# lucidrains/transfusion-pytorch

Hardware: NVIDIA H100
Metric: train tokens/sec (text+latent) at d=512 L=8 seq=1024 (higher is better)
Workload: dtype bf16

## Files before the change

transfusion_pytorch_b200/csrc/gemm_sm90.cuh:

```cuda
#pragma once
#include "sm90_ptx.cuh"
#include "dropout.cuh"

namespace tfx {

constexpr int GEMM_BM = 128;
constexpr int GEMM_BN = 128;
constexpr int GEMM_BK = 64;
constexpr int GEMM_UK = 16;

enum : int { EPI_STORE = 0, EPI_QKVG = 1, EPI_RESID = 2, EPI_GEGLU = 3, EPI_GEGLU_DROP = 4 };

struct GemmParams {
  int M, N, K;
  int k_splits;
  float* out_f32; long long ld_f32;
  __nv_bfloat16* out_bf16; long long ld_bf16;
  const float* bias;
  const long long* row_off;
  float alpha;
  int accumulate_f32;
  int K1;
  int H;
  __nv_bfloat16 *q, *k, *v;
  float* gates;
  float* mix_pre;
  float* qk_inv;
  const float *q_gamma, *k_gamma;
  const int* rope_pos;
  const float2* rope_cs;
  int rope_len;
  const int* kv_rows;
  const float* x_res; float* x_out; __nv_bfloat16* x_out_bf16;
  __nv_bfloat16* y_bf16;
  const int* cond_row;
  const float* zgate;
  long long zgate_ld;
  const float* ls;
  __nv_bfloat16* vg;
  __nv_bfloat16* h;
  DropParams drop;
};

template <int EPI> struct GemmCfg {
  static constexpr int THREADS = 384;
  static constexpr int STAGES = 4;
  static constexpr int A_BYTES = GEMM_BM * GEMM_BK * 2;
  static constexpr int B_BYTES = GEMM_BN * GEMM_BK * 2;
  static constexpr int STAGE_BYTES = A_BYTES + B_BYTES;
  static constexpr int ACC_BYTES = GEMM_BM * GEMM_BN * 4;
  static constexpr int STG_WARP = EPI == 2 ? 4096 + 2048 : 4096;
  static constexpr int STAGING = (EPI >= 3 ? 8 : 4) * STG_WARP;
  static constexpr int SMEM_BYTES = STAGES * STAGE_BYTES + ACC_BYTES + STAGING + 1024  + 256 ;
  static_assert(SMEM_BYTES <= 227 * 1024, "shared memory of one block");
};

__device__ __forceinline__ uint32_t acc_off(int r, int col) { return r * 512 + ((((col >> 2) ^ (r & 7))) << 4) + (col & 3) * 4; }
__device__ __forceinline__ void acc_ld32(const uint8_t* acc, int r, int col, uint32_t (&v)[32]) {
#pragma unroll
  for (int q = 0; q < 8; ++q) {
    const uint4 t = *reinterpret_cast<const uint4*>(acc + r * 512 + ((((col >> 2) + q) ^ (r & 7)) << 4));
    v[4 * q] = t.x; v[4 * q + 1] = t.y; v[4 * q + 2] = t.z; v[4 * q + 3] = t.w;
  }
}

__device__ __forceinline__ void gelu_parts(float g, float& cdf, float& pdf) {
  const float ax = fabsf(g) * 0.70710678118654752f;
  const float t = __fdividef(1.f, fmaf(0.3275911f, ax, 1.f));
  const float E = __expf(-ax * ax);
  float poly = fmaf(1.061405429f, t, -1.453152027f);
  poly = fmaf(poly, t, 1.421413741f);
  poly = fmaf(poly, t, -0.284496736f);
  poly = fmaf(poly, t, 0.254829592f);
  const float h = 0.5f * poly * t * E;
  cdf = g >= 0.f ? 1.f - h : h;
  pdf = 0.3989422804014327f * E;
}
__device__ __forceinline__ float gelu_erf(float x) { float c, d; gelu_parts(x, c, d); return x * c; }
__device__ __forceinline__ float2 geglu_pair(float2 g, float2 v) {
  return make_float2(gelu_erf(g.x) * v.x, gelu_erf(g.y) * v.y);
}

__device__ __forceinline__ void cp_async16_zfill(void* smem, const void* gmem, bool valid) {
  const int sz = valid ? 16 : 0;
  asm volatile("cp.async.cg.shared.global [%0], [%1], 16, %2;" ::"r"(smem_u32(smem)), "l"(gmem), "r"(sz) : "memory");
}

__device__ __forceinline__ uint32_t pack_bf16(float a, float b) {
  __nv_bfloat162 t = __floats2bfloat162_rn(a, b);
  return *reinterpret_cast<uint32_t*>(&t);
}
__device__ __forceinline__ float2 unpack2_bf16_(uint32_t w) {
  __nv_bfloat162 t = *reinterpret_cast<__nv_bfloat162*>(&w);
  return __bfloat1622float2(t);
}

template <int CH>
__device__ __forceinline__ void stg_put(uint8_t* sw, int lane, const uint32_t* w) {
#pragma unroll
  for (int c = 0; c < CH; ++c)
    *reinterpret_cast<uint4*>(sw + lane * 128 + ((c ^ (lane & 7)) << 4)) = make_uint4(w[4 * c], w[4 * c + 1], w[4 * c + 2], w[4 * c + 3]);
}
template <int CH>
__device__ __forceinline__ void stg_get(const uint8_t* sw, int lane, uint32_t* w) {
#pragma unroll
  for (int c = 0; c < CH; ++c) {
    const uint4 t = *reinterpret_cast<const uint4*>(sw + lane * 128 + ((c ^ (lane & 7)) << 4));
    w[4 * c] = t.x; w[4 * c + 1] = t.y; w[4 * c + 2] = t.z; w[4 * c + 3] = t.w;
  }
}
template <int CH>
__device__ __forceinline__ void stg_store(const uint8_t* sw, int lane, uint8_t* g, long long pitch, int rows_valid) {
  constexpr int RPI = 32 / CH;
#pragma unroll
  for (int it = 0; it < 32 / RPI; ++it) {
    const int row = it * RPI + lane / CH, ch = lane % CH;
    if (row < rows_valid)
      *reinterpret_cast<uint4*>(g + row * pitch + ch * 16) = *reinterpret_cast<const uint4*>(sw + row * 128 + ((ch ^ (row & 7)) << 4));
  }
}
__device__ __forceinline__ void stg_fetch(int lane, const uint8_t* g, long long pitch, int rows_valid, uint4 (&t)[8]) {
#pragma unroll
  for (int it = 0; it < 8; ++it) {
    const int row = it * 4 + lane / 8, ch = lane % 8;
    t[it] = row < rows_valid ? *reinterpret_cast<const uint4*>(g + row * pitch + ch * 16) : make_uint4(0, 0, 0, 0);
  }
}
__device__ __forceinline__ void stg_fill(uint8_t* sw, int lane, const uint4 (&t)[8]) {
#pragma unroll
  for (int it = 0; it < 8; ++it) {
    const int row = it * 4 + lane / 8, ch = lane % 8;
    *reinterpret_cast<uint4*>(sw + row * 128 + ((ch ^ (row & 7)) << 4)) = t[it];
  }
}

__device__ __forceinline__ void stg_put_pack(uint8_t* sw, int lane, const float* y) {
#pragma unroll
  for (int c = 0; c < 4; ++c)
    *reinterpret_cast<uint4*>(sw + lane * 128 + ((c ^ (lane & 7)) << 4)) =
        make_uint4(pack_bf16(y[8 * c], y[8 * c + 1]), pack_bf16(y[8 * c + 2], y[8 * c + 3]), pack_bf16(y[8 * c + 4], y[8 * c + 5]), pack_bf16(y[8 * c + 6], y[8 * c + 7]));
}
__device__ __forceinline__ void stg64_put(uint8_t* sw, int lane, const uint32_t* w) {
#pragma unroll
  for (int c = 0; c < 4; ++c)
    *reinterpret_cast<uint4*>(sw + lane * 64 + ((c ^ ((lane >> 1) & 3)) << 4)) = make_uint4(w[4 * c], w[4 * c + 1], w[4 * c + 2], w[4 * c + 3]);
}
__device__ __forceinline__ void stg64_put_pack(uint8_t* sw, int lane, const float* y) {
#pragma unroll
  for (int c = 0; c < 4; ++c)
    *reinterpret_cast<uint4*>(sw + lane * 64 + ((c ^ ((lane >> 1) & 3)) << 4)) =
        make_uint4(pack_bf16(y[8 * c], y[8 * c + 1]), pack_bf16(y[8 * c + 2], y[8 * c + 3]), pack_bf16(y[8 * c + 4], y[8 * c + 5]), pack_bf16(y[8 * c + 6], y[8 * c + 7]));
}
__device__ __forceinline__ void stg64_store(const uint8_t* sw, int lane, uint8_t* g, long long pitch, int rows_valid) {
#pragma unroll
  for (int it = 0; it < 4; ++it) {
    const int row = it * 8 + (lane >> 2), ch = lane & 3;
    if (row < rows_valid)
      *reinterpret_cast<uint4*>(g + row * pitch + ch * 16) = *reinterpret_cast<const uint4*>(sw + row * 64 + ((ch ^ ((row >> 1) & 3)) << 4));
  }
}

__device__ __forceinline__ void stg64_store_rows(const uint8_t* sw, int lane, uint8_t* g, long long pitch, int rows_valid, const int* __restrict__ rows) {
#pragma unroll
  for (int it = 0; it < 4; ++it) {
    const int row = it * 8 + (lane >> 2), ch = lane & 3;
    if (row < rows_valid)
      *reinterpret_cast<uint4*>(g + (long long)rows[row] * pitch + ch * 16) = *reinterpret_cast<const uint4*>(sw + row * 64 + ((ch ^ ((row >> 1) & 3)) << 4));
  }
}
template <int CH>
__device__ __forceinline__ void stg_store_rows(const uint8_t* sw, int lane, uint8_t* g, long long pitch, int rows_valid, const int* __restrict__ rows) {
  constexpr int RPI = 32 / CH;
#pragma unroll
  for (int it = 0; it < 32 / RPI; ++it) {
    const int row = it * RPI + lane / CH, ch = lane % CH;
    if (row < rows_valid)
      *reinterpret_cast<uint4*>(g + (long long)rows[row] * pitch + ch * 16) = *reinterpret_cast<const uint4*>(sw + row * 128 + ((ch ^ (row & 7)) << 4));
  }
}

template <bool A_MN, bool B_MN, int EPI, int CL>
__global__ void __launch_bounds__(384, 1)
gemm_sm90_kernel(const __grid_constant__ CUtensorMap tmA, const __grid_constant__ CUtensorMap tmA2, const __grid_constant__ CUtensorMap tmB, const GemmParams p) {
  using Cfg = GemmCfg<EPI>;
  constexpr bool GEGLU = EPI == EPI_GEGLU || EPI == EPI_GEGLU_DROP;
  constexpr int BN = GEMM_BN;
  constexpr int STAGES = Cfg::STAGES;
  static_assert(Cfg::STAGE_BYTES % 1024 == 0 && 2 * STAGES <= 32, "stage alignment / barrier area");
  extern __shared__ __align__(1024) uint8_t smem_raw[];
  uint8_t* smem = smem_raw;
  if (threadIdx.x == 0 && (smem_u32(smem) & 1023u) != 0) __trap();
  uint8_t* acc = smem + STAGES * Cfg::STAGE_BYTES;
  uint8_t* staging = acc + Cfg::ACC_BYTES;
  uint64_t* bars = reinterpret_cast<uint64_t*>(staging + Cfg::STAGING);
  uint64_t* full_bar = bars;
  uint64_t* empty_bar = bars + STAGES;

  const int warp = threadIdx.x >> 5, lane = threadIdx.x & 31;
  const int m_tiles = (p.M + GEMM_BM - 1) / GEMM_BM;
  const int n_tiles = (p.N + BN - 1) / BN;
  const int kb_total = (p.K + GEMM_BK - 1) / GEMM_BK;
  const int kb_per_split = (kb_total + p.k_splits - 1) / p.k_splits;
  const int m_units = (m_tiles + CL - 1) / CL;
  const int unit_items = m_units * n_tiles;
  const int num_items = unit_items * p.k_splits;
  const int cta_rank = CL > 1 ? (int)cluster_ctarank() : 0;
  const int first_item = blockIdx.x / CL, item_stride = gridDim.x / CL;

  if (threadIdx.x == 0) {
    tma_prefetch_desc(&tmA);
    tma_prefetch_desc(&tmB);
    for (int s = 0; s < STAGES; ++s) { mbar_init(&full_bar[s], 1); mbar_init(&empty_bar[s], 4 * CL); }
    mbar_fence_init();
  }
  __syncthreads();
  if constexpr (CL > 1) cluster_sync_all();

  if (warp < 4) {
    setmaxnreg_dec<40>();
    if (threadIdx.x == 0) {
      int stage = 0; uint32_t phase = 0;
      for (int item = first_item; item < num_items; item += item_stride) {
        const int split = item / unit_items;
        const int rem = item - split * unit_items;
        const int m_unit = rem / n_tiles, n_blk = rem - m_unit * n_tiles;
        const int m_blk = m_unit * CL + cta_rank;
        const int kb0 = split * kb_per_split;
        const int kb1 = min(kb0 + kb_per_split, kb_total);
        for (int kb = kb0; kb < kb1; ++kb) {
          mbar_wait(&empty_bar[stage], phase ^ 1);
          uint8_t* sA = smem + stage * Cfg::STAGE_BYTES;
          uint8_t* sB = sA + Cfg::A_BYTES;
          mbar_expect_tx(&full_bar[stage], Cfg::STAGE_BYTES);
          if (!A_MN) {
            if (kb * GEMM_BK < p.K1) tma_load_2d(&tmA, &full_bar[stage], sA, kb * GEMM_BK, m_blk * GEMM_BM);
            else tma_load_2d(&tmA2, &full_bar[stage], sA, kb * GEMM_BK - p.K1, m_blk * GEMM_BM);
          } else {
#pragma unroll
            for (int a = 0; a < GEMM_BM / 64; ++a)
              tma_load_2d(&tmA, &full_bar[stage], sA + a * (GEMM_BK * 128), m_blk * GEMM_BM + a * 64, kb * GEMM_BK);
          }
          if constexpr (CL > 1) {
            if (!B_MN) tma_load_2d_multicast(&tmB, &full_bar[stage], sB + cta_rank * (64 * 128), kb * GEMM_BK, n_blk * BN + cta_rank * 64, (uint16_t)3);
            else tma_load_2d_multicast(&tmB, &full_bar[stage], sB + cta_rank * (GEMM_BK * 128), n_blk * BN + cta_rank * 64, kb * GEMM_BK, (uint16_t)3);
          } else if (!B_MN) {
            tma_load_2d(&tmB, &full_bar[stage], sB, kb * GEMM_BK, n_blk * BN);
          } else {
#pragma unroll
            for (int a = 0; a < BN / 64; ++a)
              tma_load_2d(&tmB, &full_bar[stage], sB + a * (GEMM_BK * 128), n_blk * BN + a * 64, kb * GEMM_BK);
          }
          if (++stage == STAGES) { stage = 0; phase ^= 1; }
        }
      }
    }
  } else {
    setmaxnreg_inc<232>();
    constexpr int BAR_TILE = 1, BAR_MMA = 3, BAR_ACC = 5;
    const int cw = (warp >> 2) - 1;
    const int quad = warp & 3;
    uint8_t* sw = staging + ((GEGLU ? 4 * cw : 0) + quad) * Cfg::STG_WARP;
    const int erow = quad * 32 + lane;
    int stage = 0; uint32_t phase = 0;
    auto release = [&](int s) {
      __syncwarp();
      if (lane == 0) {
        if constexpr (CL > 1) { mbar_arrive_cluster(&empty_bar[s], 0); mbar_arrive_cluster(&empty_bar[s], 1); }
        else mbar_arrive(&empty_bar[s]);
      }
    };
    int nth = 0;
    for (int item = first_item; item < num_items; item += item_stride, ++nth) {
      const int split = item / unit_items;
      const int rem = item - split * unit_items;
      const int m_unit = rem / n_tiles, n_blk = rem - m_unit * n_tiles;
      const int m_blk = m_unit * CL + cta_rank;
      const int kb0 = split * kb_per_split;
      const int kb1 = min(kb0 + kb_per_split, kb_total);
      if ((nth & 1) != cw) {
        const int s = stage + (kb1 - kb0);
        stage = s % STAGES;
        phase ^= (uint32_t)(s / STAGES) & 1u;
        continue;
      }
      const bool has_next = item + item_stride < num_items;
      if (nth > 0) named_bar_sync(BAR_MMA + cw, 256);
      float d0[64], d1[64];
#pragma unroll
      for (int i = 0; i < 64; ++i) { d0[i] = 0.f; d1[i] = 0.f; }
      int prev_stage = -1;
      for (int kb = kb0; kb < kb1; ++kb) {
        mbar_wait(&full_bar[stage], phase);
        const uint32_t sA = smem_u32(smem + stage * Cfg::STAGE_BYTES);
        const uint32_t sB = sA + Cfg::A_BYTES;
        wgmma_reg_fence(d0);
        wgmma_reg_fence(d1);
        wgmma_fence();
#pragma unroll
        for (int k = 0; k < GEMM_BK / GEMM_UK; ++k) {
          const uint64_t db = B_MN ? wgmma_desc_sw128(sB + k * (GEMM_UK * 128), GEMM_BK * 128, 1024)
                                   : wgmma_desc_sw128(sB + k * (GEMM_UK * 2), 16, 1024);
          const uint64_t da0 = A_MN ? wgmma_desc_sw128(sA + k * (GEMM_UK * 128), GEMM_BK * 128, 1024)
                                    : wgmma_desc_sw128(sA + k * (GEMM_UK * 2), 16, 1024);
          const uint64_t da1 = A_MN ? wgmma_desc_sw128(sA + GEMM_BK * 128 + k * (GEMM_UK * 128), GEMM_BK * 128, 1024)
                                    : wgmma_desc_sw128(sA + 64 * 128 + k * (GEMM_UK * 2), 16, 1024);
          const uint32_t acc_flag = (kb > kb0 || k > 0) ? 1u : 0u;
          wgmma_m64n128_ss<A_MN ? 1 : 0, B_MN ? 1 : 0>(d0, da0, db, acc_flag);
          wgmma_m64n128_ss<A_MN ? 1 : 0, B_MN ? 1 : 0>(d1, da1, db, acc_flag);
        }
        wgmma_commit();
        wgmma_wait<1>();
        if (prev_stage >= 0) release(prev_stage);
        prev_stage = stage;
        if (++stage == STAGES) { stage = 0; phase ^= 1; }
      }
      if (has_next) named_bar_arrive(BAR_MMA + (cw ^ 1), 256);
      wgmma_wait<0>();
      wgmma_reg_fence(d0);
      wgmma_reg_fence(d1);
      if (prev_stage >= 0) release(prev_stage);

      if (nth > 0) named_bar_sync(BAR_ACC + cw, 256);
      {
        const int r0 = quad * 16 + (lane >> 2);
#pragma unroll
        for (int q = 0; q < 16; ++q) {
          const int c = 8 * q + 2 * (lane & 3);
          *reinterpret_cast<float2*>(acc + acc_off(r0, c)) = make_float2(d0[4 * q], d0[4 * q + 1]);
          *reinterpret_cast<float2*>(acc + acc_off(r0 + 8, c)) = make_float2(d0[4 * q + 2], d0[4 * q + 3]);
          *reinterpret_cast<float2*>(acc + acc_off(r0 + 64, c)) = make_float2(d1[4 * q], d1[4 * q + 1]);
          *reinterpret_cast<float2*>(acc + acc_off(r0 + 72, c)) = make_float2(d1[4 * q + 2], d1[4 * q + 3]);
        }
      }
      named_bar_sync(BAR_TILE + cw, 128);

      const int wrow0 = m_blk * GEMM_BM + quad * 32;
      const int row = wrow0 + lane;
      const bool row_ok = row < p.M;
      const int rows_valid = min(32, p.M - wrow0);
      const int col0 = n_blk * BN;
      int qk_pos = 0;
      if constexpr (EPI == EPI_QKVG) { qk_pos = row_ok ? p.rope_pos[row] : 0; }
      if constexpr (EPI == EPI_RESID) { qk_pos = (row_ok && p.cond_row) ? p.cond_row[row] : -1; }

      if constexpr (EPI == EPI_STORE) {
        const bool f32_staged = p.out_f32 && (p.row_off || (p.ld_f32 & 3) == 0) && ((reinterpret_cast<uintptr_t>(p.out_f32) & 15) == 0);
        const bool bf16_staged = p.out_bf16 && (p.ld_bf16 & 7) == 0 && ((reinterpret_cast<uintptr_t>(p.out_bf16) & 15) == 0);
#pragma unroll 1
        for (int c = 0; c < BN / 32; ++c) {
          const int cbase = col0 + c * 32;
          if (cbase >= p.N) break;
          uint32_t r[32];
          acc_ld32(acc, erow, c * 32, r);
          const bool full = cbase + 32 <= p.N;
          float v[32];
#pragma unroll
          for (int j = 0; j < 32; ++j) v[j] = __uint_as_float(r[j]);
          if (p.alpha != 1.f) {
#pragma unroll
            for (int j = 0; j < 32; ++j) v[j] *= p.alpha;
          }
          if (p.bias) {
            if (full) {
#pragma unroll
              for (int j = 0; j < 32; j += 4) { const float4 b = *reinterpret_cast<const float4*>(p.bias + cbase + j); v[j] += b.x; v[j + 1] += b.y; v[j + 2] += b.z; v[j + 3] += b.w; }
            } else {
              for (int j = 0; j < 32; ++j) if (cbase + j < p.N) v[j] += p.bias[cbase + j];
            }
          }
          if (p.out_f32) {
            if (full && f32_staged) {
#pragma unroll
              for (int j = 0; j < 32; ++j) r[j] = __float_as_uint(v[j]);
              stg_put<8>(sw, lane, r);
              __syncwarp();
#pragma unroll
              for (int it = 0; it < 8; ++it) {
                const int rr = it * 4 + (lane >> 3), ch = lane & 7;
                if (rr < rows_valid) {
                  const long long off = p.row_off ? p.row_off[wrow0 + rr] : (long long)(wrow0 + rr) * p.ld_f32;
                  if (off >= 0) {
                    float* dst = p.out_f32 + off + cbase + ch * 4;
                    const float4 t = *reinterpret_cast<const float4*>(sw + rr * 128 + ((ch ^ (rr & 7)) << 4));
                    if ((reinterpret_cast<uintptr_t>(dst) & 15) == 0) {
                      if (p.accumulate_f32) asm volatile("red.global.add.v4.f32 [%0], {%1, %2, %3, %4};" ::"l"(dst), "f"(t.x), "f"(t.y), "f"(t.z), "f"(t.w) : "memory");
                      else *reinterpret_cast<float4*>(dst) = t;
                    } else {
                      if (p.accumulate_f32) { atomicAdd(dst, t.x); atomicAdd(dst + 1, t.y); atomicAdd(dst + 2, t.z); atomicAdd(dst + 3, t.w); }
                      else { dst[0] = t.x; dst[1] = t.y; dst[2] = t.z; dst[3] = t.w; }
                    }
                  }
                }
              }
              __syncwarp();
            } else if (row_ok) {
              const long long off = p.row_off ? p.row_off[row] : (long long)row * p.ld_f32;
              if (off >= 0) {
                float* dst = p.out_f32 + off + cbase;
                for (int j = 0; j < 32; ++j)
                  if (cbase + j < p.N) { if (p.accumulate_f32) atomicAdd(dst + j, v[j]); else dst[j] = v[j]; }
              }
            }
          }
          if (p.out_bf16) {
            if (full && bf16_staged) {
              uint32_t w[16];
#pragma unroll
              for (int j = 0; j < 16; ++j) w[j] = pack_bf16(v[2 * j], v[2 * j + 1]);
              stg_put<4>(sw, lane, w);
              __syncwarp();
              stg_store<4>(sw, lane, reinterpret_cast<uint8_t*>(p.out_bf16 + (long long)wrow0 * p.ld_bf16 + cbase), p.ld_bf16 * 2, rows_valid);
              __syncwarp();
            } else if (row_ok) {
              __nv_bfloat16* dst = p.out_bf16 + (long long)row * p.ld_bf16 + cbase;
              for (int j = 0; j < 32; ++j) if (cbase + j < p.N) dst[j] = __float2bfloat16(v[j]);
            }
          }
        }
      } else if constexpr (EPI == EPI_QKVG) {
        const int tps = p.H >> 1;
        const int kind = n_blk / tps;
        const int tis = n_blk - kind * tps;
        const long long HI = (long long)p.H * 64;
        if (kind <= 1) {
          const float* gamma = kind == 0 ? p.q_gamma : p.k_gamma;
          __nv_bfloat16* dstm = kind == 0 ? p.q : p.k;
          const float2* cs = p.rope_cs + qk_pos;
#pragma unroll
          for (int hh = 0; hh < 2; ++hh) {
            uint32_t r0[32], r1[32];
            acc_ld32(acc, erow, hh * 64, r0);
            acc_ld32(acc, erow, hh * 64 + 32, r1);
            float ss = 0.f;
#pragma unroll
            for (int j = 0; j < 32; ++j) { float a = __uint_as_float(r0[j]), b = __uint_as_float(r1[j]); ss += a * a + b * b; }
            const float inv = 1.f / fmaxf(sqrtf(ss), 1e-12f);
            const int head = tis * 2 + hh;
            if (row_ok) p.qk_inv[(long long)row * 2 * p.H + kind * p.H + head] = inv;
            const float sc = inv * 8.f;
            uint32_t outw[32];
#pragma unroll
            for (int dh = 0; dh < 2; ++dh) {
              uint32_t* rr = dh == 0 ? r0 : r1;
#pragma unroll
              for (int i = 0; i < 16; ++i) {
                const int d0 = dh * 32 + 2 * i;
                const float2 gm = *reinterpret_cast<const float2*>(gamma + d0);
                const float y0 = __uint_as_float(rr[2 * i]) * sc * (gm.x + 1.f);
                const float y1 = __uint_as_float(rr[2 * i + 1]) * sc * (gm.y + 1.f);
                const float2 cc = cs[(long long)(dh * 16 + i) * p.rope_len];
                outw[dh * 16 + i] = pack_bf16(y0 * cc.x - y1 * cc.y, y1 * cc.x + y0 * cc.y);
              }
            }
            stg_put<8>(sw, lane, outw);
            __syncwarp();
            if (kind == 1 && p.kv_rows) stg_store_rows<8>(sw, lane, reinterpret_cast<uint8_t*>(dstm + head * 64), HI * 2, rows_valid, p.kv_rows + wrow0);
            else stg_store<8>(sw, lane, reinterpret_cast<uint8_t*>(dstm + (long long)wrow0 * HI + head * 64), HI * 2, rows_valid);
            __syncwarp();
          }
        } else if (kind == 2) {
#pragma unroll
          for (int c = 0; c < 2; ++c) {
            uint32_t r0[32], r1[32], w[32];
            acc_ld32(acc, erow, c * 64, r0);
            acc_ld32(acc, erow, c * 64 + 32, r1);
#pragma unroll
            for (int j = 0; j < 16; ++j) {
              w[j] = pack_bf16(__uint_as_float(r0[2 * j]), __uint_as_float(r0[2 * j + 1]));
              w[16 + j] = pack_bf16(__uint_as_float(r1[2 * j]), __uint_as_float(r1[2 * j + 1]));
            }
            stg_put<8>(sw, lane, w);
            __syncwarp();
            if (p.kv_rows) stg_store_rows<8>(sw, lane, reinterpret_cast<uint8_t*>(p.v + tis * 128 + c * 64), HI * 2, rows_valid, p.kv_rows + wrow0);
            else stg_store<8>(sw, lane, reinterpret_cast<uint8_t*>(p.v + (long long)wrow0 * HI + tis * 128 + c * 64), HI * 2, rows_valid);
            __syncwarp();
          }
        } else {
          uint32_t r[32];
          acc_ld32(acc, erow, 0, r);
          if (row_ok) {
            float* dst = p.gates + (long long)row * p.H;
#pragma unroll
            for (int j = 0; j < 32; ++j) if (j < p.H) dst[j] = __uint_as_float(r[j]);
            if (p.mix_pre) {
              float* dm = p.mix_pre + (long long)row * p.H;
#pragma unroll
              for (int j = 0; j < 32; ++j) if (j >= p.H && j < 2 * p.H) dm[j - p.H] = __uint_as_float(r[j]);
            }
          }
        }
      } else if constexpr (EPI == EPI_RESID) {
        const int crow = qk_pos;
        const float* zrow = (p.zgate && crow >= 0) ? p.zgate + (long long)crow * p.zgate_ld : nullptr;
        uint8_t* swb = sw + 4096;
        uint4 xres[8];
        auto fetch = [&](int sl) {
          stg_fetch(lane, reinterpret_cast<const uint8_t*>(p.x_res + (long long)wrow0 * p.N + col0 + sl * 32), (long long)p.N * 4,
                    col0 + sl * 32 < p.N ? rows_valid : 0, xres);
        };
        fetch(0);
#pragma unroll 1
        for (int sl = 0; sl < BN / 32; ++sl) {
          const int cbase = col0 + sl * 32;
          if (cbase >= p.N) break;
          __syncwarp();
          stg_fill(sw, lane, xres);
          if (sl + 1 < BN / 32) fetch(sl + 1);
          uint32_t r[32];
          acc_ld32(acc, erow, sl * 32, r);
          float y[32];
#pragma unroll
          for (int j = 0; j < 32; ++j) y[j] = __uint_as_float(r[j]);
          if (p.bias) {
#pragma unroll
            for (int j = 0; j < 32; j += 4) { const float4 b = *reinterpret_cast<const float4*>(p.bias + cbase + j); y[j] += b.x; y[j + 1] += b.y; y[j + 2] += b.z; y[j + 3] += b.w; }
          }
          if (p.y_bf16) {
            stg64_put_pack(swb, lane, y);
            __syncwarp();
            stg64_store(swb, lane, reinterpret_cast<uint8_t*>(p.y_bf16 + (long long)wrow0 * p.N + cbase), (long long)p.N * 2, rows_valid);
            __syncwarp();
          }
          {
            uint32_t xrv[32];
            __syncwarp();
            stg_get<8>(sw, lane, xrv);
            if (zrow) {
#pragma unroll
              for (int j = 0; j < 32; j += 4) {
                const float4 s4 = *reinterpret_cast<const float4*>(zrow + cbase + j);
                y[j] = __uint_as_float(xrv[j]) + y[j] * s4.x; y[j + 1] = __uint_as_float(xrv[j + 1]) + y[j + 1] * s4.y;
                y[j + 2] = __uint_as_float(xrv[j + 2]) + y[j + 2] * s4.z; y[j + 3] = __uint_as_float(xrv[j + 3]) + y[j + 3] * s4.w;
              }
            } else if (p.ls) {
#pragma unroll
              for (int j = 0; j < 32; j += 4) {
                const float4 s4 = *reinterpret_cast<const float4*>(p.ls + cbase + j);
                y[j] = __uint_as_float(xrv[j]) + y[j] * (s4.x + 1.f); y[j + 1] = __uint_as_float(xrv[j + 1]) + y[j + 1] * (s4.y + 1.f);
                y[j + 2] = __uint_as_float(xrv[j + 2]) + y[j + 2] * (s4.z + 1.f); y[j + 3] = __uint_as_float(xrv[j + 3]) + y[j + 3] * (s4.w + 1.f);
              }
            } else {
#pragma unroll
              for (int j = 0; j < 32; ++j) y[j] += __uint_as_float(xrv[j]);
            }
          }
          if (p.x_out)
#pragma unroll
          for (int hfc = 0; hfc < 2; ++hfc) {
            uint32_t w16[16];
#pragma unroll
            for (int j = 0; j < 16; ++j) w16[j] = __float_as_uint(y[hfc * 16 + j]);
            __syncwarp();
            stg64_put(swb, lane, w16);
            __syncwarp();
            stg64_store(swb, lane, reinterpret_cast<uint8_t*>(p.x_out + (long long)wrow0 * p.N + cbase + hfc * 16), (long long)p.N * 4, rows_valid);
          }
          if (p.x_out_bf16) {
            __syncwarp();
            stg64_put_pack(swb, lane, y);
            __syncwarp();
            stg64_store(swb, lane, reinterpret_cast<uint8_t*>(p.x_out_bf16 + (long long)wrow0 * p.N + cbase), (long long)p.N * 2, rows_valid);
          }
          __syncwarp();
        }
      } else if constexpr (GEGLU) {
        uint32_t keep[2] = {0u, 0u};
        if constexpr (EPI == EPI_GEGLU_DROP) {
          const uint32_t k0 = __ldg(p.drop.key), k1 = __ldg(p.drop.key + 1);
#pragma unroll
          for (int q = 0; q < 8; ++q) keep[q >> 2] |= drop_keep8(p.drop, k0, k1, DROP_SITE_FFN, 0, (uint32_t)row, (uint32_t)(n_blk * 8 + q)) << (8 * (q & 3));
        }
        uint32_t ra[4][32];
#pragma unroll
        for (int q = 0; q < 4; ++q) acc_ld32(acc, erow, q * 32, ra[q]);
        if (has_next) named_bar_arrive(BAR_ACC + (cw ^ 1), 256);
#pragma unroll
        for (int c = 0; c < 2; ++c) {
          const int cv = col0 + c * 32, cg = cv + 64;
          if (cv >= p.N) break;
          float v[32], g[32];
#pragma unroll
          for (int j = 0; j < 32; ++j) { v[j] = __uint_as_float(ra[c][j]) + p.bias[cv + j]; g[j] = __uint_as_float(ra[2 + c][j]) + p.bias[cg + j]; }
          __syncwarp();
          stg64_put_pack(sw, lane, v);
          __syncwarp();
          stg64_store(sw, lane, reinterpret_cast<uint8_t*>(p.vg + (long long)wrow0 * p.N + cv), (long long)p.N * 2, rows_valid);
          __syncwarp();
          stg64_put_pack(sw, lane, g);
          __syncwarp();
          stg64_store(sw, lane, reinterpret_cast<uint8_t*>(p.vg + (long long)wrow0 * p.N + cg), (long long)p.N * 2, rows_valid);
#pragma unroll
          for (int j = 0; j < 32; j += 2) {
            const float2 o = geglu_pair(make_float2(g[j], g[j + 1]), make_float2(v[j], v[j + 1]));
            g[j] = o.x; g[j + 1] = o.y;
          }
          if constexpr (EPI == EPI_GEGLU_DROP) {
#pragma unroll
            for (int j = 0; j < 32; ++j) g[j] = (keep[c] >> j) & 1u ? g[j] * p.drop.scale : 0.f;
          }
          __syncwarp();
          stg64_put_pack(sw, lane, g);
          __syncwarp();
          stg64_store(sw, lane, reinterpret_cast<uint8_t*>(p.h + (long long)wrow0 * (p.N / 2) + n_blk * 64 + c * 32), (long long)p.N, rows_valid);
          __syncwarp();
        }
      }
      if (!GEGLU && has_next) named_bar_arrive(BAR_ACC + (cw ^ 1), 256);
    }
  }
  if constexpr (CL > 1) {
    __syncthreads();
    cluster_sync_all();
  }
}

typedef CUresult (*PFN_encodeTiled)(CUtensorMap*, CUtensorMapDataType, cuuint32_t, void*, const cuuint64_t*, const cuuint64_t*,
                                    const cuuint32_t*, const cuuint32_t*, CUtensorMapInterleave, CUtensorMapSwizzle,
                                    CUtensorMapL2promotion, CUtensorMapFloatOOBfill);

inline PFN_encodeTiled get_encode_fn() {
  static PFN_encodeTiled fn = nullptr;
  if (!fn) {
    void* f = nullptr;
    cudaDriverEntryPointQueryResult qres;
    if (cudaGetDriverEntryPoint("cuTensorMapEncodeTiled", &f, cudaEnableDefault, &qres) != cudaSuccess || !f) return nullptr;
    fn = reinterpret_cast<PFN_encodeTiled>(f);
  }
  return fn;
}

inline int make_tmap_bf16(CUtensorMap* tm, const void* ptr, long long inner, long long outer, long long ld, int box_rows) {
  PFN_encodeTiled enc = get_encode_fn();
  if (!enc) return -1;
  cuuint64_t dims[2] = {(cuuint64_t)inner, (cuuint64_t)outer};
  cuuint64_t strides[1] = {(cuuint64_t)ld * 2};
  cuuint32_t box[2] = {64, (cuuint32_t)box_rows};
  cuuint32_t estr[2] = {1, 1};
  CUresult r = enc(tm, CU_TENSOR_MAP_DATA_TYPE_BFLOAT16, 2, const_cast<void*>(ptr), dims, strides, box, estr,
                   CU_TENSOR_MAP_INTERLEAVE_NONE, CU_TENSOR_MAP_SWIZZLE_128B, CU_TENSOR_MAP_L2_PROMOTION_L2_256B,
                   CU_TENSOR_MAP_FLOAT_OOB_FILL_NONE);
  return r == CUDA_SUCCESS ? 0 : -(int)r - 1000;
}

struct GemmOperand {
  const void* ptr;
  long long ld;
  bool mn_major;
  const void* ptr2 = nullptr;
  long long ld2 = 0;
};

inline int& gemm_cluster_mode_ref() {
  static int mode = -1;
  if (mode < 0) { const char* e = getenv("TFX_GEMM_CLUSTER"); mode = e ? atoi(e) : 1; }
  return mode;
}

template <bool A_MN, bool B_MN, int EPI>
int launch_gemm_t(const GemmOperand& A, const GemmOperand& B, const GemmParams& p_in, int num_sms, cudaStream_t stream) {
  using Cfg = GemmCfg<EPI>;
  GemmParams p = p_in;
  CUtensorMap tmA, tmA2, tmB;
  int rc;
  const bool two = (!A_MN) && A.ptr2 != nullptr;
  if (!two) p.K1 = p.K;
  if (!A_MN) rc = make_tmap_bf16(&tmA, A.ptr, two ? p.K1 : p.K, p.M, A.ld, GEMM_BM); else rc = make_tmap_bf16(&tmA, A.ptr, p.M, p.K, A.ld, GEMM_BK);
  if (rc) return rc;
  if (two) { rc = make_tmap_bf16(&tmA2, A.ptr2, p.K - p.K1, p.M, A.ld2, GEMM_BM); if (rc) return rc; } else tmA2 = tmA;
  {
    const int kbt = (p.K + GEMM_BK - 1) / GEMM_BK;
    if (p.k_splits < 1) p.k_splits = 1;
    if (p.k_splits > kbt) p.k_splits = kbt;
    const int per = (kbt + p.k_splits - 1) / p.k_splits;
    p.k_splits = (kbt + per - 1) / per;
  }
  const int m_tiles = (p.M + GEMM_BM - 1) / GEMM_BM, n_tiles = (p.N + GEMM_BN - 1) / GEMM_BN;
  const int items = m_tiles * n_tiles * p.k_splits;
  if (items <= 0) return 0;
  const int mode = gemm_cluster_mode_ref();
  const int kb_item = ((p.K + GEMM_BK - 1) / GEMM_BK + p.k_splits - 1) / p.k_splits;
  const bool paired = mode == 2 || (mode == 3 && m_tiles >= 2 && kb_item >= 16 && items >= 2 * num_sms);
  if (!B_MN) rc = make_tmap_bf16(&tmB, B.ptr, p.K, p.N, B.ld, paired ? GEMM_BN / 2 : GEMM_BN); else rc = make_tmap_bf16(&tmB, B.ptr, p.N, p.K, B.ld, GEMM_BK);
  if (rc) return rc;
  if (paired) {
    auto kern = gemm_sm90_kernel<A_MN, B_MN, EPI, 2>;
    static int max_clusters = 0;
    cudaLaunchConfig_t cfg;
    memset(&cfg, 0, sizeof(cfg));
    cudaLaunchAttribute at[1];
    at[0].id = cudaLaunchAttributeClusterDimension;
    at[0].val.clusterDim.x = 2; at[0].val.clusterDim.y = 1; at[0].val.clusterDim.z = 1;
    cfg.blockDim = dim3(Cfg::THREADS); cfg.dynamicSmemBytes = Cfg::SMEM_BYTES; cfg.stream = stream; cfg.attrs = at; cfg.numAttrs = 1;
    if (!max_clusters) {
      if (cudaFuncSetAttribute(kern, cudaFuncAttributeMaxDynamicSharedMemorySize, Cfg::SMEM_BYTES) != cudaSuccess) return -2;
      cfg.gridDim = dim3(2 * (num_sms / 2));
      int nc = 0;
      if (cudaOccupancyMaxActiveClusters(&nc, kern, &cfg) != cudaSuccess || nc < 1) { cudaGetLastError(); nc = num_sms / 2; }
      max_clusters = nc < num_sms / 2 ? nc : num_sms / 2;
    }
    const int pair_items = ((m_tiles + 1) / 2) * n_tiles * p.k_splits;
    const int clusters = pair_items < max_clusters ? pair_items : max_clusters;
    cfg.gridDim = dim3(2 * clusters);
    return cudaLaunchKernelEx(&cfg, kern, tmA, tmA2, tmB, p) == cudaSuccess ? 0 : -3;
  }
  auto kern = gemm_sm90_kernel<A_MN, B_MN, EPI, 1>;
  static bool attr_set = false;
  if (!attr_set) {
    if (cudaFuncSetAttribute(kern, cudaFuncAttributeMaxDynamicSharedMemorySize, Cfg::SMEM_BYTES) != cudaSuccess) return -2;
    attr_set = true;
  }
  const int grid = items < num_sms ? items : num_sms;
  kern<<<grid, Cfg::THREADS, Cfg::SMEM_BYTES, stream>>>(tmA, tmA2, tmB, p);
  return cudaGetLastError() == cudaSuccess ? 0 : -3;
}

}
```

transfusion_pytorch_b200/csrc/sm90_ptx.cuh:

```cuda
#pragma once
#include <cuda.h>
#include <cuda_runtime.h>
#include <cuda_bf16.h>
#include <stdint.h>
#include <stdio.h>

namespace tfx {

#ifndef TFX_SPIN_LIMIT
#define TFX_SPIN_LIMIT (1u << 24)
#endif

__device__ __forceinline__ uint32_t smem_u32(const void* p) {
  return static_cast<uint32_t>(__cvta_generic_to_shared(p));
}

__device__ __forceinline__ void mbar_init(uint64_t* bar, uint32_t count) {
  asm volatile("mbarrier.init.shared::cta.b64 [%0], %1;" ::"r"(smem_u32(bar)), "r"(count));
}
__device__ __forceinline__ void mbar_fence_init() {
  asm volatile("fence.mbarrier_init.release.cluster;" ::: "memory");
}
__device__ __forceinline__ void mbar_expect_tx(uint64_t* bar, uint32_t bytes) {
  asm volatile("mbarrier.arrive.expect_tx.shared::cta.b64 _, [%0], %1;" ::"r"(smem_u32(bar)), "r"(bytes) : "memory");
}
__device__ __forceinline__ void mbar_arrive(uint64_t* bar) {
  asm volatile("mbarrier.arrive.shared::cta.b64 _, [%0];" ::"r"(smem_u32(bar)) : "memory");
}
__device__ __forceinline__ bool mbar_try_wait(uint64_t* bar, uint32_t parity) {
  uint32_t ok;
  asm volatile(
      "{\n\t.reg .pred p;\n\t"
      "mbarrier.try_wait.parity.shared::cta.b64 p, [%1], %2;\n\t"
      "selp.u32 %0, 1, 0, p;\n\t}"
      : "=r"(ok) : "r"(smem_u32(bar)), "r"(parity) : "memory");
  return ok != 0;
}
__device__ __forceinline__ void mbar_wait(uint64_t* bar, uint32_t parity) {
  uint32_t spins = 0;
  while (!mbar_try_wait(bar, parity)) {
    if (++spins > TFX_SPIN_LIMIT) {
#if defined(TFX_DEBUG_SPIN) && TFX_DEBUG_SPIN
      printf("tfx: mbarrier timeout block %d thread %d bar %u parity %u\n", blockIdx.x, threadIdx.x, smem_u32(bar), parity);
#endif
      __trap();
    }
  }
}

__device__ __forceinline__ void tma_prefetch_desc(const CUtensorMap* m) {
  asm volatile("prefetch.tensormap [%0];" ::"l"(reinterpret_cast<uint64_t>(m)) : "memory");
}
__device__ __forceinline__ void tma_load_2d(const CUtensorMap* m, uint64_t* bar, void* smem, int c0, int c1) {
  asm volatile(
      "cp.async.bulk.tensor.2d.shared::cluster.global.mbarrier::complete_tx::bytes [%0], [%1, {%3, %4}], [%2];"
      ::"r"(smem_u32(smem)), "l"(reinterpret_cast<uint64_t>(m)), "r"(smem_u32(bar)), "r"(c0), "r"(c1)
      : "memory");
}
__device__ __forceinline__ void tma_load_1d(const CUtensorMap* m, uint64_t* bar, void* smem, int c0) {
  asm volatile(
      "cp.async.bulk.tensor.1d.shared::cluster.global.mbarrier::complete_tx::bytes [%0], [%1, {%3}], [%2];"
      ::"r"(smem_u32(smem)), "l"(reinterpret_cast<uint64_t>(m)), "r"(smem_u32(bar)), "r"(c0)
      : "memory");
}
__device__ __forceinline__ void tma_reduce_add_2d(const CUtensorMap* m, const void* smem, int c0, int c1) {
  asm volatile("cp.reduce.async.bulk.tensor.2d.global.shared::cta.add.tile.bulk_group [%0, {%2, %3}], [%1];"
               ::"l"(reinterpret_cast<uint64_t>(m)), "r"(smem_u32(smem)), "r"(c0), "r"(c1) : "memory");
}
__device__ __forceinline__ void bulk_commit() { asm volatile("cp.async.bulk.commit_group;" ::: "memory"); }
__device__ __forceinline__ void bulk_wait_read_all() { asm volatile("cp.async.bulk.wait_group.read 0;" ::: "memory"); }
__device__ __forceinline__ void bulk_wait_all() { asm volatile("cp.async.bulk.wait_group 0;" ::: "memory"); }
__device__ __forceinline__ void tma_load_2d_multicast(const CUtensorMap* m, uint64_t* bar, void* smem, int c0, int c1, uint16_t mask) {
  asm volatile(
      "cp.async.bulk.tensor.2d.shared::cluster.global.mbarrier::complete_tx::bytes.multicast::cluster [%0], [%1, {%3, %4}], [%2], %5;"
      ::"r"(smem_u32(smem)), "l"(reinterpret_cast<uint64_t>(m)), "r"(smem_u32(bar)), "r"(c0), "r"(c1), "h"(mask)
      : "memory");
}
__device__ __forceinline__ uint32_t cluster_ctarank() { uint32_t r; asm volatile("mov.u32 %0, %%cluster_ctarank;" : "=r"(r)); return r; }
__device__ __forceinline__ void cluster_sync_all() {
  asm volatile("barrier.cluster.arrive.release.aligned;\n\tbarrier.cluster.wait.acquire.aligned;" ::: "memory");
}
__device__ __forceinline__ void mbar_arrive_cluster(uint64_t* bar, uint32_t rank) {
  uint32_t remote;
  asm volatile("mapa.shared::cluster.u32 %0, %1, %2;" : "=r"(remote) : "r"(smem_u32(bar)), "r"(rank));
  asm volatile("mbarrier.arrive.release.cluster.shared::cluster.b64 _, [%0];" ::"r"(remote) : "memory");
}
__device__ __forceinline__ void fence_proxy_async_smem() {
  asm volatile("fence.proxy.async.shared::cta;" ::: "memory");
}
__device__ __forceinline__ void named_bar_sync(int id, int count) {
  asm volatile("bar.sync %0, %1;" ::"r"(id), "r"(count) : "memory");
}
__device__ __forceinline__ void named_bar_arrive(int id, int count) {
  asm volatile("bar.arrive %0, %1;" ::"r"(id), "r"(count) : "memory");
}

template <int N> __device__ __forceinline__ void setmaxnreg_dec() { asm volatile("setmaxnreg.dec.sync.aligned.u32 %0;" ::"n"(N)); }
template <int N> __device__ __forceinline__ void setmaxnreg_inc() { asm volatile("setmaxnreg.inc.sync.aligned.u32 %0;" ::"n"(N)); }

__device__ __forceinline__ void wgmma_fence() { asm volatile("wgmma.fence.sync.aligned;" ::: "memory"); }
__device__ __forceinline__ void wgmma_commit() { asm volatile("wgmma.commit_group.sync.aligned;" ::: "memory"); }
template <int N> __device__ __forceinline__ void wgmma_wait() { asm volatile("wgmma.wait_group.sync.aligned %0;" ::"n"(N) : "memory"); }
template <int N> __device__ __forceinline__ void wgmma_reg_fence(float (&d)[N]) {
#pragma unroll
  for (int i = 0; i < N; ++i) asm volatile("" : "+f"(d[i])::"memory");
}

template <int TA, int TB>
__device__ __forceinline__ void wgmma_m64n128_ss(float (&d)[64], uint64_t da, uint64_t db, uint32_t accumulate) {
  asm volatile(
      "{\n\t.reg .pred p;\n\t"
      "setp.ne.b32 p, %66, 0;\n\t"
      "wgmma.mma_async.sync.aligned.m64n128k16.f32.bf16.bf16 "
      "{%0, %1, %2, %3, %4, %5, %6, %7, %8, %9, %10, %11, %12, %13, %14, %15, %16, %17, %18, %19, %20, %21, %22, %23, %24, %25, %26, %27, %28, %29, %30, %31, %32, %33, %34, %35, %36, %37, %38, %39, %40, %41, %42, %43, %44, %45, %46, %47, %48, %49, %50, %51, %52, %53, %54, %55, %56, %57, %58, %59, %60, %61, %62, %63}, "
      "%64, %65, p, 1, 1, %67, %68;\n\t}"
      : "+f"(d[0]), "+f"(d[1]), "+f"(d[2]), "+f"(d[3]), "+f"(d[4]), "+f"(d[5]), "+f"(d[6]), "+f"(d[7]), "+f"(d[8]), "+f"(d[9]), "+f"(d[10]), "+f"(d[11]), "+f"(d[12]), "+f"(d[13]), "+f"(d[14]), "+f"(d[15]), "+f"(d[16]), "+f"(d[17]), "+f"(d[18]), "+f"(d[19]), "+f"(d[20]), "+f"(d[21]), "+f"(d[22]), "+f"(d[23]), "+f"(d[24]), "+f"(d[25]), "+f"(d[26]), "+f"(d[27]), "+f"(d[28]), "+f"(d[29]), "+f"(d[30]), "+f"(d[31]), "+f"(d[32]), "+f"(d[33]), "+f"(d[34]), "+f"(d[35]), "+f"(d[36]), "+f"(d[37]), "+f"(d[38]), "+f"(d[39]), "+f"(d[40]), "+f"(d[41]), "+f"(d[42]), "+f"(d[43]), "+f"(d[44]), "+f"(d[45]), "+f"(d[46]), "+f"(d[47]), "+f"(d[48]), "+f"(d[49]), "+f"(d[50]), "+f"(d[51]), "+f"(d[52]), "+f"(d[53]), "+f"(d[54]), "+f"(d[55]), "+f"(d[56]), "+f"(d[57]), "+f"(d[58]), "+f"(d[59]), "+f"(d[60]), "+f"(d[61]), "+f"(d[62]), "+f"(d[63])
      : "l"(da), "l"(db), "r"(accumulate), "n"(TA), "n"(TB));
}
template <int TA, int TB>
__device__ __forceinline__ void wgmma_m64n64_ss(float (&d)[32], uint64_t da, uint64_t db, uint32_t accumulate) {
  asm volatile(
      "{\n\t.reg .pred p;\n\t"
      "setp.ne.b32 p, %34, 0;\n\t"
      "wgmma.mma_async.sync.aligned.m64n64k16.f32.bf16.bf16 "
      "{%0, %1, %2, %3, %4, %5, %6, %7, %8, %9, %10, %11, %12, %13, %14, %15, %16, %17, %18, %19, %20, %21, %22, %23, %24, %25, %26, %27, %28, %29, %30, %31}, "
      "%32, %33, p, 1, 1, %35, %36;\n\t}"
      : "+f"(d[0]), "+f"(d[1]), "+f"(d[2]), "+f"(d[3]), "+f"(d[4]), "+f"(d[5]), "+f"(d[6]), "+f"(d[7]), "+f"(d[8]), "+f"(d[9]), "+f"(d[10]), "+f"(d[11]), "+f"(d[12]), "+f"(d[13]), "+f"(d[14]), "+f"(d[15]), "+f"(d[16]), "+f"(d[17]), "+f"(d[18]), "+f"(d[19]), "+f"(d[20]), "+f"(d[21]), "+f"(d[22]), "+f"(d[23]), "+f"(d[24]), "+f"(d[25]), "+f"(d[26]), "+f"(d[27]), "+f"(d[28]), "+f"(d[29]), "+f"(d[30]), "+f"(d[31])
      : "l"(da), "l"(db), "r"(accumulate), "n"(TA), "n"(TB));
}
template <int TB>
__device__ __forceinline__ void wgmma_m64n64_rs(float (&d)[32], const uint32_t (&a)[4], uint64_t db, uint32_t accumulate) {
  asm volatile(
      "{\n\t.reg .pred p;\n\t"
      "setp.ne.b32 p, %37, 0;\n\t"
      "wgmma.mma_async.sync.aligned.m64n64k16.f32.bf16.bf16 "
      "{%0, %1, %2, %3, %4, %5, %6, %7, %8, %9, %10, %11, %12, %13, %14, %15, %16, %17, %18, %19, %20, %21, %22, %23, %24, %25, %26, %27, %28, %29, %30, %31}, "
      "{%32, %33, %34, %35}, %36, p, 1, 1, %38;\n\t}"
      : "+f"(d[0]), "+f"(d[1]), "+f"(d[2]), "+f"(d[3]), "+f"(d[4]), "+f"(d[5]), "+f"(d[6]), "+f"(d[7]), "+f"(d[8]), "+f"(d[9]), "+f"(d[10]), "+f"(d[11]), "+f"(d[12]), "+f"(d[13]), "+f"(d[14]), "+f"(d[15]), "+f"(d[16]), "+f"(d[17]), "+f"(d[18]), "+f"(d[19]), "+f"(d[20]), "+f"(d[21]), "+f"(d[22]), "+f"(d[23]), "+f"(d[24]), "+f"(d[25]), "+f"(d[26]), "+f"(d[27]), "+f"(d[28]), "+f"(d[29]), "+f"(d[30]), "+f"(d[31])
      : "r"(a[0]), "r"(a[1]), "r"(a[2]), "r"(a[3]), "l"(db), "r"(accumulate), "n"(TB));
}

__device__ __forceinline__ uint64_t wgmma_desc_sw128(uint32_t smem_addr, uint32_t lbo_bytes, uint32_t sbo_bytes) {
  uint64_t d = 0;
  d |= (uint64_t)((smem_addr >> 4) & 0x3FFF);
  d |= (uint64_t)((lbo_bytes >> 4) & 0x3FFF) << 16;
  d |= (uint64_t)((sbo_bytes >> 4) & 0x3FFF) << 32;
  d |= (uint64_t)1 << 62;
  return d;
}

}
```

transfusion_pytorch_b200/engine.py:

```python
from __future__ import annotations

import math
import os
import ctypes
from dataclasses import dataclass

import numpy as np
import torch
from torch import Tensor

from . import _lib
from ._pinned import POOL
from .modality_processing import RaggedBatch

BF16, F32, I32, I64 = torch.bfloat16, torch.float32, torch.int32, torch.int64


def _round_up(x: int, m: int) -> int:
    return (x + m - 1) // m * m


_EMPTY_I32 = np.zeros(0, dtype = np.int32)


def posemb_tables(params, lens, device):
    out = []
    for (w0, b0, w2, b2), L in zip(params, lens):
        seq = torch.arange(int(L), device = device, dtype = F32)[:, None]
        pre = seq * w0.reshape(1, -1) + b0
        act = pre * torch.sigmoid(pre)
        out.append((seq, pre, act, act @ w2.t() + b2))
    return out


def posemb_add(rows: Tensor, tables, coords):
    for (_, _, _, e), c in zip(tables, coords):
        rows += e.index_select(0, c)


def posemb_backward(d_rows: Tensor, tables, coords, params, grads):
    for (seq, pre, act, e), c, (w0, b0, w2, b2), (gw0, gb0, gw2, gb2) in zip(tables, coords, params, grads):
        d_e = torch.zeros_like(e).index_add_(0, c, d_rows)
        gw2 += d_e.t() @ act
        gb2 += d_e.sum(0)
        sig = torch.sigmoid(pre)
        d_pre = (d_e @ w2) * (sig * (1. + pre * (1. - sig)))
        gw0 += (d_pre * seq).sum(0)[:, None]
        gb0 += d_pre.sum(0)


class KVCache:

    def __init__(self, engine, n_slabs: int, cap: int):
        self.n_slabs, self.cap, self.rows = int(n_slabs), int(cap), int(n_slabs) * int(cap)
        nbytes = 2 * engine.depth * self.rows * engine.HI * 2
        assert nbytes < 96 << 30, f'kv cache of {nbytes / 2**30:.1f} GiB requested ({n_slabs} slabs x {cap} rows): lower max_length / batch the prompts'
        self.k = torch.zeros(engine.depth, self.rows, engine.HI, device = engine.device, dtype = BF16)
        self.v = torch.zeros(engine.depth, self.rows, engine.HI, device = engine.device, dtype = BF16)
        self.vl = torch.zeros_like(self.v) if engine.laser else None

    def slab_start(self, s):
        return np.asarray(s, dtype = np.int64) * self.cap


class Engine:
    def __init__(self, model):
        self.ops = _lib.Ops()
        self.model = model
        tr = model.transformer
        self.D, self.H, self.depth = tr.dim, tr.heads, tr.depth
        self.HI = self.H * 64
        self.inner = tr.ff_inner
        self.Ip = _round_up(self.inner, 64)
        self.NQ = 3 * self.HI + 128
        self.V = model.text_embed.weight.shape[0]
        self.Vp = _round_up(self.V, 8)
        self.Kt = _round_up(self.D + 1, 64)
        self.W = 2 * self.depth
        self.softcap = tr.softcap_value
        self.laser, self.laser_clamp, self.vres = tr.attn_laser, tr.laser_softclamp_value, tr.use_value_residual
        self.clean, self.clean_eps = bool(getattr(model, 'model_output_clean', False)), float(getattr(model, 'eps', 1e-2))
        self.posemb = tuple(bool(a) for a in getattr(model, 'add_pos_emb', ()))
        self.scale = 64 ** -0.5
        self.dls = list(model.dim_latents)
        self.dlp = [_round_up(d, 8) for d in self.dls]
        assert self.D % 128 == 0 and self.D <= 1024, 'model dim must be a multiple of 128 and <= 1024 for the row kernels'
        assert self.H % 2 == 0 and 2 <= self.H <= 32, 'heads must be even (two 64-wide heads per 128-column GEMM tile)'
        self.device = None
        self.flat = None
        self.ws = {}
        self._dirty = True
        self._ptr_arrays = []
        self.launches = 0
        self.graph_pins = None
        self.hid_bf16 = os.environ.get('TFX_HIDDEN_BF16', '1') == '1'
        self.ares_deferred = self.hid_bf16 and os.environ.get('TFX_ARES_DEFERRED', '1') == '1'
        self.frozen = False

    def _trainable(self):
        m = self.model
        skip = set()
        for mod in list(m.modality_encoder) + list(m.modality_decoder):
            if mod is not None:
                skip |= {id(p) for p in mod.parameters()}
        return [(n, p) for n, p in m.named_parameters() if p.requires_grad and id(p) not in skip]

    def attach(self):
        named = self._trainable()
        late = lambda n: ('.to_film.' in n) or ('.to_ada_ln_zero.' in n) or n.startswith('transformer.to_time_cond.')
        named = [(n, p) for n, p in named if not late(n)] + [(n, p) for n, p in named if late(n)]
        dev = named[0][1].device
        if dev.type != 'cuda':
            raise _lib.TfxError(f'the CUDA engine needs the model on a CUDA device (got {dev}); there is no CPU path')
        rc = self.ops.lib.tfx_init(dev.index if dev.index is not None else torch.cuda.current_device())
        _lib.check(rc, 'tfx_init')
        self.device = dev
        offs, total = {}, 0
        for n, p in named:
            offs[n] = total
            total += _round_up(p.numel(), 4)
        flat = torch.zeros(total, device = dev, dtype = F32)
        gflat = torch.zeros(total, device = dev, dtype = F32)
        for n, p in named:
            o, k = offs[n], p.numel()
            flat[o:o + k].copy_(p.data.reshape(-1).float())
            p.data = flat[o:o + k].view(p.shape)
            p.grad = gflat[o:o + k].view(p.shape)
        self.flat, self.gflat, self.offs, self.named = flat, gflat, offs, dict(named)
        self.named_first = named[0][1]
        self.exp_avg = self.exp_avg_sq = None
        self.opt_step = 0
        self._first_ptr = named[0][1].data_ptr()
        self.late_start = min((offs[n] for n, _ in named if late(n)), default = total)
        self._build_maps()
        self._dirty = True
        if not getattr(self, '_hooked', False):
            self.model.register_load_state_dict_post_hook(lambda *a, **k: self.mark_dirty())
            self._hooked = True

    def mark_dirty(self):
        self._dirty = True

    def ensure_attached(self):
        if self.flat is None or self.named_first.data_ptr() != self._first_ptr:
            self.attach()

    def P(self, name):
        return self.named[name]

    def _posemb_params(self, t, nax, grads = False):
        get = self.G if grads else self.P
        return [tuple(get(f'pos_emb_mlp.{t}.mlps.{a}.{k}') for k in ('0.weight', '0.bias', '2.weight', '2.bias')) for a in range(nax)]

    def G(self, name):
        o, p = self.offs[name], self.named[name]
        return self.gflat[o:o + p.numel()].view(p.shape)

    def _build_maps(self):
        dev, D, HI, H, inner, Ip = self.device, self.D, self.HI, self.H, self.inner, self.Ip
        src = np.full(2 * Ip, -1, dtype = np.int64)
        for t in range(Ip // 64):
            for j in range(64):
                c = 64 * t + j
                if c < inner:
                    src[128 * t + j] = c
                    src[128 * t + 64 + j] = inner + c
        self.w1_row_src = torch.from_numpy(src.astype(np.int32)).to(dev)
        self.w1_row_src64 = torch.from_numpy(src).to(dev)
        self.layer_maps = []
        for i in range(self.depth):
            pre = f'transformer.layers.{i}'
            w1_off = self.offs[f'{pre}.2.fn.net.0.weight']
            b1_off = self.offs[f'{pre}.2.fn.net.0.bias']
            w1_rows = torch.where(self.w1_row_src64 >= 0, w1_off + self.w1_row_src64 * D, torch.full_like(self.w1_row_src64, -1))
            b1_cols = torch.where(self.w1_row_src64 >= 0, b1_off + self.w1_row_src64, torch.full_like(self.w1_row_src64, -1)).to(I32)
            q_off, v_off, g_off = self.offs[f'{pre}.1.fn.to_qk.0.weight'], self.offs[f'{pre}.1.fn.to_v.0.weight'], self.offs[f'{pre}.1.fn.to_gates.0.weight']
            r = np.full(self.NQ, -1, dtype = np.int64)
            r[:2 * HI] = q_off + np.arange(2 * HI) * D
            r[2 * HI:3 * HI] = v_off + np.arange(HI) * D
            r[3 * HI:3 * HI + H] = g_off + np.arange(H) * D
            if f'{pre}.1.fn.to_learned_value_residual.0.weight' in self.offs:
                r[3 * HI + H:3 * HI + 2 * H] = self.offs[f'{pre}.1.fn.to_learned_value_residual.0.weight'] + np.arange(H) * D
            w2_off = self.offs[f'{pre}.2.fn.net.3.weight']
            w2_rows = torch.from_numpy(w2_off + np.arange(D, dtype = np.int64) * inner).to(dev)
            self.layer_maps.append(dict(w1_rows = w1_rows.contiguous(), b1_cols = b1_cols.contiguous(), qkvg_rows = torch.from_numpy(r).to(dev), w2_rows = w2_rows))
        rows = np.full(self.W * 3 * D, -1, dtype = np.int64)
        bias_idx = np.zeros(self.W * 3 * D, dtype = np.int64)
        for w in range(self.W):
            i, j = divmod(w, 2)
            pre = f'transformer.layers.{i}.{j + 1}'
            fo, zo = self.offs[f'{pre}.to_film.weight'], self.offs[f'{pre}.to_ada_ln_zero.weight']
            rows[w * 3 * D: w * 3 * D + 2 * D] = fo + np.arange(2 * D) * 4 * D
            rows[w * 3 * D + 2 * D: (w + 1) * 3 * D] = zo + np.arange(D) * 4 * D
            bias_idx[w * 3 * D: w * 3 * D + 2 * D] = self.offs[f'{pre}.to_film.bias'] + np.arange(2 * D)
            bias_idx[w * 3 * D + 2 * D: (w + 1) * 3 * D] = self.offs[f'{pre}.to_ada_ln_zero.bias'] + np.arange(D)
        self.fz_rows = torch.from_numpy(rows).to(dev)
        self.fz_bias_idx = torch.from_numpy(bias_idx).to(dev)
        tw = self.offs['transformer.to_time_cond.1.weight']
        self.wt_rows = torch.from_numpy(tw + np.arange(4 * D, dtype = np.int64) * (D + 1)).to(dev)

    def buf(self, name, shape, dtype, zero = False):
        t = self.ws.get(name)
        n = int(np.prod(shape)) if len(shape) else 1
        if t is None or t.dtype != dtype or t.numel() < n:
            if t is not None and self.graph_pins is not None:
                self.graph_pins.append(t)
            t = torch.empty(max(n, 1), device = self.device, dtype = dtype)
            self.ws[name] = t
            if zero:
                t.zero_()
        return t[:n].view(shape)

    def pin_workspaces(self):
        if self.graph_pins is None:
            self.graph_pins = []

    def _build_pack_jobs(self):
        D, HI, H, Ip, inner = self.D, self.HI, self.H, self.Ip, self.inner
        pk = self.packed = {}
        jobs = []
        def dst(name, rows, cols, dtype = BF16):
            t = pk[name] = torch.zeros(rows, cols, device = self.device, dtype = dtype) if cols else torch.zeros(rows, device = self.device, dtype = dtype)
            return t
        def job(src, ld_src, c_src, row_src, d, r_dst, c_dst):
            jobs.append((src, ld_src, c_src, row_src, d, r_dst, c_dst, 1 if d.dtype == F32 else 0))
        for i in range(self.depth):
            pre = f'transformer.layers.{i}'
            wq = dst(f'qkvg{i}', self.NQ, D)
            job(self.P(f'{pre}.1.fn.to_qk.0.weight'), D, D, None, wq, 2 * HI, D)
            job(self.P(f'{pre}.1.fn.to_v.0.weight'), D, D, None, wq[2 * HI:], HI, D)
            job(self.P(f'{pre}.1.fn.to_gates.0.weight'), D, D, None, wq[3 * HI:], H, D)
            if f'{pre}.1.fn.to_learned_value_residual.0.weight' in self.named:
                job(self.P(f'{pre}.1.fn.to_learned_value_residual.0.weight'), D, D, None, wq[3 * HI + H:], H, D)
            job(self.P(f'{pre}.1.fn.to_out.1.weight'), HI, HI, None, dst(f'wo{i}', D, HI), D, HI)
            job(self.P(f'{pre}.2.fn.net.0.weight'), D, D, self.w1_row_src, dst(f'w1{i}', 2 * Ip, D), 2 * Ip, D)
            job(self.P(f'{pre}.2.fn.net.3.weight'), inner, inner, None, dst(f'w2{i}', D, Ip), D, Ip)
            job(self.P(f'{pre}.2.fn.net.0.bias'), 1, 1, self.w1_row_src, dst(f'b1{i}', 2 * Ip, 0, F32), 2 * Ip, 1)
            if f'{pre}.0.weight' in self.named:
                job(self.P(f'{pre}.0.weight'), 2 * D, 2 * D, None, dst(f'wskip{i}', D, 2 * D), D, 2 * D)
        job(self.P('to_text_logits.weight'), D, D, None, dst('wvocab', self.V, D), self.V, D)
        for t, (dl, dlp) in enumerate(zip(self.dls, self.dlp)):
            job(self.P(f'model_to_latent_projs.{t}.weight'), D, D, None, dst(f'wm2l{t}', dl, D), dl, D)
            if f'latent_to_model_projs.{t}.weight' in self.named:
                job(self.P(f'latent_to_model_projs.{t}.weight'), dl, dl, None, dst(f'wl2m{t}', D, dlp), D, dlp)
        job(self.P('transformer.to_time_cond.1.weight'), D + 1, D + 1, None, dst('wt', 4 * D, self.Kt), 4 * D, self.Kt)
        wfz = dst('wfz', self.W * 3 * D, 4 * D)
        bfz = dst('bfz', self.W * 3 * D, 0, F32)
        for w in range(self.W):
            i, j = divmod(w, 2)
            pre = f'transformer.layers.{i}.{j + 1}'
            job(self.P(f'{pre}.to_film.weight'), 4 * D, 4 * D, None, wfz[w * 3 * D:], 2 * D, 4 * D)
            job(self.P(f'{pre}.to_ada_ln_zero.weight'), 4 * D, 4 * D, None, wfz[w * 3 * D + 2 * D:], D, 4 * D)
            job(self.P(f'{pre}.to_film.bias'), 2 * D, 2 * D, None, bfz[w * 3 * D:], 1, 2 * D)
            job(self.P(f'{pre}.to_ada_ln_zero.bias'), D, D, None, bfz[w * 3 * D + 2 * D:], 1, D)
        dt = np.dtype([('src', '<u8'), ('ld_src', '<i8'), ('row_src', '<u8'), ('dst', '<u8'), ('R_dst', '<i8'), ('C_src', '<i4'), ('C_dst', '<i4'),
                       ('dst_f32', '<i4'), ('pad', '<i4')])
        assert dt.itemsize == 56
        tab = np.zeros(len(jobs), dtype = dt)
        blk_job, blk_first = [], []
        for j, (src, ld_src, c_src, row_src, d, r_dst, c_dst, f32) in enumerate(jobs):
            tab[j] = (src.data_ptr(), ld_src, row_src.data_ptr() if row_src is not None else 0, d.data_ptr(), r_dst, c_src, c_dst, f32, 0)
            nb = (r_dst * c_dst + 2047) // 2048
            blk_first.append(len(blk_job))
            blk_job.extend([j] * nb)
        self._pack_tab = torch.from_numpy(tab.view(np.uint8).copy()).to(self.device)
        self._pack_blk_job = torch.tensor(blk_job, dtype = I32, device = self.device)
        self._pack_blk_first = torch.tensor(blk_first, dtype = I32, device = self.device)
        self._pack_nblocks = len(blk_job)
        self._pack_ptr = self._first_ptr

    def pack_weights(self, force = False):
        have = getattr(self, 'packed', None) is not None and getattr(self, '_pack_ptr', None) == self._first_ptr
        if have and not self._dirty and (self.frozen or not force):
            return
        if getattr(self, '_pack_ptr', None) != self._first_ptr:
            self._build_pack_jobs()
        self.ops.cast_pack_multi(self._pack_tab, self._pack_blk_job, self._pack_blk_first, self._pack_nblocks)
        if getattr(self, 'fastp', None) is None or self.fastp.device != self.device:
            self.fastp = torch.zeros(self.depth, 8, device = self.device, dtype = F32)
        for i in range(self.depth):
            pre = f'transformer.layers.{i}.1.fn'
            self.ops.attn_fast_params(self.P(f'{pre}.q_norm.gamma'), self.P(f'{pre}.k_norm.gamma'), 64, self.scale, self.softcap, self.fastp[i])
        self._dirty = False

    META_NAMES = ['text_id', 'label', 'kv_limit', 'rope_pos', 'cond_row', 'slot', 'tile_q0', 'tile_qend', 'tile_kv0', 'tile_kvend',
                  'kt_kv0', 'kt_kvend', 'kt_q0', 'kt_qend', 'row_token', 't2_q0', 't2_qend', 't2_kv0', 't2_kvend', 'k2_kv0', 'k2_kvend', 'k2_q0', 'k2_qend', 'k2_order', 'kv_row', 'pos_c0', 'pos_c1', 'pos_c2']

    def stage_meta(self, rb: RaggedBatch):
        ints = [getattr(rb, n) if getattr(rb, n) is not None else _EMPTY_I32 for n in self.META_NAMES]
        sizes = [_round_up(a.shape[0], 4) for a in ints]
        fl = np.concatenate([rb.cond_times, rb.row_time]).astype(np.float32)
        n_int, n_fl = sum(sizes), _round_up(fl.shape[0], 4)
        raw = POOL.take((n_int + n_fl) * 4)
        host = raw[:(n_int + n_fl) * 4].view(I32)
        hv = host.numpy()
        off = 0
        for a, s in zip(ints, sizes):
            hv[off:off + a.shape[0]] = a; off += s
        hv[n_int:n_int + fl.shape[0]] = fl.view(np.int32)
        return raw, host, (tuple(a.shape[0] for a in ints), tuple(sizes), n_int, fl.shape[0])

    def meta_views(self, rb: RaggedBatch, devbuf: Tensor, layout):
        lens, sizes, n_int, n_fl = layout
        d, off = {}, 0
        for n, ln, s in zip(self.META_NAMES, lens, sizes):
            d[n] = devbuf[off:off + ln]; off += s
        fdev = devbuf[n_int:n_int + n_fl].view(F32)
        d['cond_times'], d['row_time'] = fdev[:rb.n_cond], fdev[rb.n_cond:]
        d['h2d_bytes'] = devbuf.numel() * 4
        d['_keep'] = devbuf
        d['_layout'] = layout
        return d

    def upload(self, rb: RaggedBatch):
        if rb.dev:
            return rb.dev
        raw, host, layout = self.stage_meta(rb)
        devbuf = host.to(self.device, non_blocking = True)
        POOL.give(raw)
        rb.dev = self.meta_views(rb, devbuf, layout)
        return rb.dev

    def rope_table(self, max_pos: int):
        n = _round_up(max_pos + 1, 1024)
        t = self.ws.get('rope_cs')
        if t is None or t.shape[0] < n:
            if t is not None and self.graph_pins is not None:
                self.graph_pins += [t, self.ws['rope_cs_t']]
            t = torch.empty(n, 32, 2, device = self.device, dtype = F32)
            tt = torch.empty(32, n, 2, device = self.device, dtype = F32)
            self.ops.rope_table(self.model.rotary_emb.freqs.detach().float().contiguous(), t, tt, n, 32)
            self.ws['rope_cs'], self.ws['rope_cs_t'] = t, tt
        return t

    def _ptr_array(self, tensors):
        arr = (ctypes.c_void_p * len(tensors))(*[t.data_ptr() for t in tensors])
        self._ptr_arrays.append(arr)
        if len(self._ptr_arrays) > 256:
            self._ptr_arrays = self._ptr_arrays[-64:]
        return ctypes.cast(arr, ctypes.c_void_p)

    def forward(self, rb: RaggedBatch, latents: list | None, eps: list | None, *, train: bool, want_logits = False, vlimit = 0,
                text_loss_weight = 1., flow_loss_weight = 1., modality_only = False, cache: KVCache | None = None, want_preds = None,
                vel_targets = None, vel_weight = 0., dropout = False, dropout_key = None):
        self.ensure_attached()
        self.pack_weights(force = train)
        o, D, HI, H, Ip, M = self.ops, self.D, self.HI, self.H, self.Ip, rb.M
        dv = self.upload(rb)
        nc, S = rb.n_cond, rb.S
        p_ff = self.model.transformer.ff_dropout_p(train, dropout)
        st = self.state = dict(rb = rb, train = train, layers = [], p_ff = p_ff, drop_key = self.dropout_key(dropout_key) if p_ff > 0. else None)
        pk = self.packed
        rope = self.rope_table(rb.max_rope_pos)
        cond_row = dv['cond_row'] if nc > 0 else None
        tag = 'T' if train else 'I'
        assert cache is None or not train, 'the kv cache is an inference-time structure'
        kv_rows = dv['kv_row'] if cache is not None else None
        M_kv = cache.rows if cache is not None else 0
        want_preds = want_logits if want_preds is None else want_preds

        if nc > 0:
            feats = self.buf('feats', (nc, self.Kt), BF16)
            o.time_features(dv['cond_times'], self.model.transformer.to_time_cond[0].weights, feats, nc, D // 2, self.Kt)
            cpre = self.buf('cpre', (nc, 4 * D), F32)
            o.gemm_store(feats, self.Kt, 0, pk['wt'], self.Kt, 0, nc, 4 * D, self.Kt, cpre, 4 * D, None, 0, self.P('transformer.to_time_cond.1.bias'), None, 1.0, 0, 1)
            cond = self.buf('cond', (nc, 4 * D), BF16)
            o.table_op(cpre, 4 * D, None, 0, None, 0, cond, 4 * D, nc, 4 * D, 1)
            tab = self.buf('tab', (nc, self.W * 3 * D), F32)
            o.gemm_store(cond, 4 * D, 0, pk['wfz'], 4 * D, 0, nc, self.W * 3 * D, 4 * D, tab, self.W * 3 * D, None, 0, pk['bfz'], None, 1.0, 0, 1)
            zg = self.buf('zg', (nc, self.W * D), F32)
            for w in range(self.W):
                o.table_op(tab[:, w * 3 * D + 2 * D:], self.W * 3 * D, None, 0, zg[:, w * D:], self.W * D, None, 0, nc, D, 0)
            st.update(feats = feats, cpre = cpre, cond = cond, tab = tab, zg = zg)
        tab_ld, zg_ld = self.W * 3 * D, self.W * D

        modtok = None
        if S > 0:
            modtok = self.buf('modtok', (S, D), F32)
            st['noised'], st['flow'] = [], []
            for t, (s0, s1) in enumerate(rb.type_rows):
                n = s1 - s0
                if n == 0:
                    st['noised'].append(None); st['flow'].append(None); continue
                dl, dlp = self.dls[t], self.dlp[t]
                x = latents[t]
                assert x.shape == (n, dl) and x.dtype == F32 and x.is_cuda, f'latents[{t}] must be a cuda fp32 [{n}, {dl}] tensor'
                noised = self.buf(f'noised{t}', (n, dlp), BF16)
                if dlp != dl:
                    noised[:, dl:].zero_()
                has_proj = f'latent_to_model_projs.{t}.weight' in self.named
                nf32 = None if has_proj else modtok[s0:s1]
                if eps is not None and eps[t] is not None:
                    flow = self.buf(f'flow{t}', (n, dl), F32)
                    o.flow_noise(x, eps[t], dv['row_time'][s0:s1], noised, dlp, nf32, flow, n, dl)
                else:
                    flow = None
                    o.flow_noise(x, None, None, noised, dlp, None, None, n, dl)
                    if not has_proj:
                        modtok[s0:s1].copy_(x)
                if has_proj:
                    o.gemm_store(noised, dlp, 0, pk[f'wl2m{t}'], dlp, 0, n, D, dl, modtok[s0:s1], D, None, 0, self.P(f'latent_to_model_projs.{t}.bias'), None, 1.0, 0, 1)
                if self.posemb and self.posemb[t]:
                    nax = int(self.model.modality_num_dim[t])
                    coords = [dv[f'pos_c{a}'][s0:s1] for a in range(nax)]
                    tabs = posemb_tables(self._posemb_params(t, nax), rb.pos_max[t][:nax], self.device)
                    posemb_add(modtok[s0:s1], tabs, coords)
                    st.setdefault('posemb', {})[t] = (tabs, coords)
                st['noised'].append(noised); st['flow'].append(flow)
        x0 = self.buf(f'{tag}x0', (M, D), F32)
        x0b = self.buf(f'{tag}x0b', (M, D), BF16)
        o.embed_assemble(dv['text_id'], self.P('text_embed.weight'), modtok, dv['slot'] if S > 0 else None, x0, x0b, M, D)

        hid = [x0b if self.hid_bf16 else x0]
        skips = []
        x_in, x_in_b = x0, x0b
        n_tiles = int(rb.tile_q0.shape[0])
        for i in range(self.depth):
            L = {}
            pre = f'transformer.layers.{i}'
            lt = f'{tag}{i}' if train else 'I'
            layer = i + 1
            first_half = layer <= self.depth // 2
            if first_half:
                skips.append((i, x_in_b))
            has_skip = (not first_half) and f'{pre}.0.weight' in self.named
            if has_skip:
                src_i, skip_b = skips.pop()
                x_a = self.buf(f'{lt}xa', (M, D), F32)
                o.gemm_resid(x_in_b, D, skip_b, D, D, pk[f'wskip{i}'], 2 * D, M, D, 2 * D, None, x_in, x_a, None, None, None, None, 0, None)
                L.update(skip_src = src_i, skip_b = skip_b)
            else:
                x_a = x_in
            wA, wF = 2 * i, 2 * i + 1
            filmA = tab[:, wA * 3 * D:] if nc > 0 else None
            filmF = tab[:, wF * 3 * D:] if nc > 0 else None
            zgA = zg[:, wA * D:] if nc > 0 else None
            zgF = zg[:, wF * D:] if nc > 0 else None
            uA = self.buf(f'{lt}uA', (M, D), BF16); statsA = self.buf(f'{lt}sA', (M, 2), F32)
            o.adaln_fwd(x_a, cond_row, filmA, tab_ld, self.P(f'{pre}.1.layernorm_gamma'), uA, statsA, M, D)
            q = self.buf(f'{lt}q', (M, HI), BF16)
            if cache is not None:
                k, v = cache.k[i], cache.v[i]
            else:
                k = self.buf(f'{lt}k', (M, HI), BF16); v = self.buf(f'{lt}v0' if (self.vres and i == 0) else f'{lt}v', (M, HI), BF16)
            gates = self.buf(f'{lt}g', (M, H), F32); qk_inv = self.buf(f'{lt}qi', (M, 2 * H), F32)
            has_mix = self.vres and i > 0
            mixpre = self.buf(f'{lt}mix', (M, H), F32) if has_mix else None
            o.gemm_qkvg(uA, D, pk[f'qkvg{i}'], D, M, H, D, q, k, v, gates, qk_inv, self.P(f'{pre}.1.fn.q_norm.gamma'), self.P(f'{pre}.1.fn.k_norm.gamma'),
                        dv['rope_pos'], self.ws['rope_cs_t'], int(self.ws['rope_cs_t'].shape[1]), kv_rows, mixpre)
            if has_mix:
                v_first = cache.v[0] if cache is not None else st['layers'][0]['v']
                o.vmix_fwd(v, HI, kv_rows, v_first, HI, mixpre, self.P(f'{pre}.1.fn.to_learned_value_residual.0.bias'), M, H)
            v_att, att_gates = v, gates
            if self.laser:
                v_att = cache.vl[i] if cache is not None else self.buf(f'{lt}vl', (M, HI), BF16)
                o.laser_v_fwd(v, HI, kv_rows, v_att, HI, M, H, self.laser_clamp)
                att_gates = None
            att = self.buf(f'{lt}o', (M, HI), BF16); lse = self.buf(f'{lt}lse', (H, M), F32)
            o_l = self.buf(f'{lt}ol', (M, HI), BF16) if self.laser else att
            fp = self.fastp[i]
            if getattr(rb, 'single_row_tiles', False):
                o.attn_decode(q, k, v_att, HI, HI, HI, att_gates, H, dv['kv_limit'], dv['tile_q0'], dv['tile_kv0'], dv['tile_kvend'], n_tiles, o_l, HI, self.scale, self.softcap)
            else:
                o.attn_fwd_tc(q, k, v_att, HI, HI, HI, att_gates, H, dv['kv_limit'], dv['t2_q0'], dv['t2_qend'], dv['t2_kv0'], dv['t2_kvend'], int(rb.t2_q0.shape[0]),
                              o_l, HI, lse, M, M_kv, self.scale, self.softcap, fp)
                o.attn_fwd(q, k, v_att, HI, HI, HI, att_gates, H, dv['kv_limit'], dv['tile_q0'], dv['tile_qend'], dv['tile_kv0'], dv['tile_kvend'], n_tiles,
                           o_l, HI, lse, M, self.scale, self.softcap, fp)
            if self.laser:
                o.laser_out_fwd(o_l, gates, att, M, H)
            x_b = self.buf(f'{lt}xb', (M, D), F32); yA = self.buf(f'{lt}yA', (M, D), BF16) if train else None
            o.gemm_resid(att, HI, None, 0, 0, pk[f'wo{i}'], HI, M, D, HI, None, x_a, x_b, None, yA, cond_row, zgA, zg_ld, self.P(f'{pre}.1.layerscale'))
            uF = self.buf(f'{lt}uF', (M, D), BF16); statsF = self.buf(f'{lt}sF', (M, 2), F32)
            o.adaln_fwd(x_b, cond_row, filmF, tab_ld, self.P(f'{pre}.2.layernorm_gamma'), uF, statsF, M, D)
            vg = self.buf(f'{lt}vg', (M, 2 * Ip), BF16); h = self.buf(f'{lt}h', (M, Ip), BF16)
            if p_ff > 0.:
                o.gemm_geglu_drop(uF, D, pk[f'w1{i}'], D, pk[f'b1{i}'], M, 2 * Ip, D, vg, h, st['drop_key'], p_ff, i)
            else:
                o.gemm_geglu(uF, D, pk[f'w1{i}'], D, pk[f'b1{i}'], M, 2 * Ip, D, vg, h)
            yF = self.buf(f'{lt}yF', (M, D), BF16) if train else None
            if self.hid_bf16:
                x_c = self.buf(f'{tag}Hb{i + 1}', (M, D), BF16)
                o.gemm_resid(h, Ip, None, 0, 0, pk[f'w2{i}'], Ip, M, D, Ip, self.P(f'{pre}.2.fn.net.3.bias'), x_b, None, x_c, yF, cond_row, zgF, zg_ld,
                             self.P(f'{pre}.2.layerscale'))
            else:
                x_c = self.buf(f'{tag}H{i + 1}', (M, D), F32)
                o.gemm_resid(h, Ip, None, 0, 0, pk[f'w2{i}'], Ip, M, D, Ip, self.P(f'{pre}.2.fn.net.3.bias'), x_b, x_c, None, yF, cond_row, zgF, zg_ld,
                             self.P(f'{pre}.2.layerscale'))
            hid.append(x_c)
            xr = self.buf(f'{tag}xr{i}', (M, D), F32); xrb = self.buf(f'{tag}xrb{i}', (M, D), BF16)
            rlse = self.buf(f'{tag}rlse{i}', (M,), F32) if train else None
            (o.attn_residual_fwd_h16 if self.hid_bf16 else o.attn_residual_fwd)(self._ptr_array(hid), len(hid), self.P(f'{pre}.3.norm_keys.gamma'), self.P(f'{pre}.3.pseudo_queries'),
                                                                                 xr, xrb, rlse, M, D)
            L.update(xr = xr, rlse = rlse, mixpre = mixpre, o_l = o_l, v_att = v_att)
            L.update(x_a = x_a, uA = uA, statsA = statsA, q = q, k = k, v = v, gates = gates, qk_inv = qk_inv, att = att, lse = lse, yA = yA, x_b = x_b,
                     uF = uF, statsF = statsF, vg = vg, h = h, yF = yF, x_in = x_in, x_in_b = x_in_b, has_skip = has_skip, first_half = first_half)
            st['layers'].append(L)
            x_in, x_in_b = xr, xrb
        st['hid'] = hid
        st['x_last'] = x_in

        out = self.buf(f'{tag}out', (M, D), F32)
        outb = self.buf(f'{tag}outb', (M, D), BF16)
        omod = self.buf(f'{tag}omod', (max(S, 1), D), BF16)
        o.rmsnorm_fwd(x_in, self.P('transformer.norm.gamma'), out, outb, dv['slot'] if S > 0 else None, omod if S > 0 else None, M, D)
        if self.clean and S > 0:
            o.clean_flow_fwd(out, dv['row_token'], modtok, dv['cond_times'], dv['cond_row'], self.clean_eps, omod, S, D)
        st.update(out = out, outb = outb, omod = omod)
        res = dict(embed = out)

        if want_logits or train:
            logits = self.buf(f'{tag}logits', (M, self.Vp), F32)
            o.gemm_store(outb, D, 0, pk['wvocab'], D, 0, M, self.V, D, logits, self.Vp, None, 0, None, None, 1.0, 0, 1)
            res['logits'] = logits
            st['logits'] = logits
        preds = []
        if S > 0 and (train or want_preds):
            for t, (s0, s1) in enumerate(rb.type_rows):
                n = s1 - s0
                if n == 0:
                    preds.append(None); continue
                dl = self.dls[t]
                pred = self.buf(f'{tag}pred{t}', (n, dl), F32)
                o.gemm_store(omod[s0:s1], D, 0, pk[f'wm2l{t}'], D, 0, n, dl, D, pred, dl, None, 0, None, None, 1.0, 0, 1)
                preds.append(pred)
            res['preds'] = preds
        if train:
            T = float(rb.total_tokens)
            acc = self.buf('lossacc', (2 + len(self.dls),), torch.float64)
            acc.zero_()
            nvalid = self.buf('nvalid', (1,), I32); nvalid.zero_()
            dlog = self.buf('dlogits', (M, self.Vp), BF16)
            if modality_only:
                dlog.zero_()
            else:
                gs = (text_loss_weight / T) if vlimit == 0 else 1.0 / max(rb.n_valid, 1)
                o.ce_fwd_bwd(logits, self.Vp, dv['label'], self.V, vlimit, gs, dlog, self.Vp, acc[0:1], nvalid, M)
            st['dlogits'] = dlog
            st['dpred'] = []
            flow_terms = []
            vel_terms = {}
            for t, (s0, s1) in enumerate(rb.type_rows):
                n = s1 - s0
                if n == 0 or st['flow'][t] is None:
                    st['dpred'].append(None); flow_terms.append(None); continue
                dl, dlp = self.dls[t], self.dlp[t]
                wt = 1.0 if modality_only else rb.n_type_tokens[t] / T
                dpred = self.buf(f'dpred{t}', (n, dlp), BF16)
                if dlp != dl:
                    dpred[:, dl:].zero_()
                ga = 2.0 * flow_loss_weight * wt / (n * dl)
                if vel_targets is not None and vel_targets[t] is not None and vel_weight != 0.:
                    e = vel_targets[t]
                    assert e.shape == (n, dl) and e.dtype == F32
                    gb = 2.0 * vel_weight * wt / (n * dl)
                    vacc = self.buf('velacc', (len(self.dls),), torch.float64)
                    if t == 0 or not vel_terms:
                        vacc.zero_()
                    o.mse_fwd_bwd(preds[t], dl, e, None, dlp, gb, vacc[t: t + 1], n, dl)
                    o.mse_fwd_bwd(preds[t], dl, st['flow'][t], None, dlp, ga, acc[1 + t: 2 + t], n, dl)
                    blend = self.buf(f'velblend{t}', (n, dl), F32)
                    blend.zero_()
                    o.axpy_f32(blend, st['flow'][t], ga / (ga + gb), n * dl)
                    o.axpy_f32(blend, e, gb / (ga + gb), n * dl)
                    scratch = self.buf('velscratch', (1,), torch.float64)
                    o.mse_fwd_bwd(preds[t], dl, blend, dpred, dlp, ga + gb, scratch, n, dl)
                    vel_terms[t] = (vacc[t] / (n * dl)).float()
                else:
                    o.mse_fwd_bwd(preds[t], dl, st['flow'][t], dpred, dlp, ga, acc[1 + t: 2 + t], n, dl)
                st['dpred'].append(dpred)
                flow_terms.append((acc[1 + t] / (n * dl)).float() )
            text = (acc[0] / nvalid[0].clamp(min = 1)).float()
            flows = torch.stack([f if f is not None else torch.zeros((), device = self.device) for f in flow_terms]) if flow_terms else torch.zeros(0, device = self.device)
            if vlimit:
                total = text.clone()
            elif modality_only:
                total = flows.sum()
            else:
                total = (acc[0] / T).float() * text_loss_weight
                for t, f in enumerate(flow_terms):
                    if f is not None:
                        total = total + f * (rb.n_type_tokens[t] / T) * flow_loss_weight
                for t, f in vel_terms.items():
                    total = total + f * (rb.n_type_tokens[t] / T) * vel_weight
            vel = [vel_terms.get(t, torch.zeros((), device = self.device)) for t in range(len(self.dls))] if vel_terms else None
            res.update(loss_acc = acc, n_valid = nvalid, total = total, text = text, flows = flows, vel = vel)
        return res

    def dropout_key(self, src = None, out: Tensor | None = None) -> Tensor:
        if torch.is_tensor(src):
            assert src.dtype == I32 and src.numel() == 2 and src.device == self.device, 'a dropout key tensor is int32 [2] on the engine device'
            return src
        key = out if out is not None else self.buf('drop_key', (2,), I32)
        if src is None:
            key.random_(-2 ** 31, 2 ** 31)
        else:
            key.copy_(torch.from_numpy(np.array(src, dtype = np.uint32).view(np.int32)))
        return key

    def _prepare_grads(self):
        missing = [(n, p) for n, p in self.named.items() if p.grad is None or p.grad.data_ptr() != self.gflat.data_ptr() + 4 * self.offs[n]]
        if not missing:
            return
        if len(missing) == len(self.named):
            self.gflat.zero_()
        for n, p in missing:
            gv = self.G(n)
            if len(missing) != len(self.named):
                gv.zero_()
            if p.grad is not None:
                gv.copy_(p.grad)
            p.grad = gv

    def backward(self, gscale = None, bucket_cb = None):
        st = self.state
        assert st['train'], 'backward() needs a train forward'
        self._prepare_grads()
        self._grads_clean = False
        self._dirty = True
        if gscale is not None:
            gs = gscale.detach().float().reshape(1)
            self.ops.scale_bf16(st['dlogits'], gs, st['dlogits'].numel())
            for dp in st['dpred']:
                if dp is not None:
                    self.ops.scale_bf16(dp, gs, dp.numel())
        rb, dv = st['rb'], st['rb'].dev
        o, D, HI, H, Ip, M, inner = self.ops, self.D, self.HI, self.H, self.Ip, st['rb'].M, self.inner
        pk, nc, S = self.packed, rb.n_cond, rb.S
        cond_row = dv['cond_row'] if nc > 0 else None
        tab_ld, zg_ld = self.W * 3 * D, self.W * D
        ks = max(1, min(64, M // 2048))
        sms = torch.cuda.get_device_properties(self.device).multi_processor_count
        def ksplit(n_out, n_in, K = M):
            tiles = ((n_out + 127) // 128) * ((n_in + 255) // 256 if (n_in % 256 == 0 or n_in >= 1024) else (n_in + 127) // 128)
            best, best_eff = 1, 0.0
            for s in range(1, 65):
                if K // s < 1024 and s > 1:
                    break
                items = tiles * s
                eff = items / (-(-items // sms) * sms)
                if eff > best_eff + 0.02 or (abs(eff - best_eff) <= 0.02 and s <= ks and s > best):
                    best, best_eff = s, eff
            return best
        def wgrad(dy, ld_dy, n_out, act, ld_act, n_in, gname, K = M):
            o.gemm_store(dy, ld_dy, 1, act, ld_act, 1, n_out, n_in, K, self.G(gname), n_in, None, 0, None, None, 1.0, 1, ksplit(n_out, n_in, K))

        dlog = st['dlogits']
        d_out = self.buf('d_out', (M, D), F32)
        o.gemm_store(dlog, self.Vp, 0, pk['wvocab'], D, 1, M, D, self.V, d_out, D, None, 0, None, None, 1.0, 0, 1)
        wgrad(dlog, self.Vp, self.V, st['outb'], D, D, 'to_text_logits.weight')
        if S > 0:
            dmod = self.buf('dmod', (S, D), F32)
            any_flow = False
            for t, (s0, s1) in enumerate(rb.type_rows):
                n = s1 - s0
                dp = st['dpred'][t] if n else None
                if dp is None:
                    if n:
                        dmod[s0:s1].zero_()
                    continue
                any_flow = True
                dl, dlp = self.dls[t], self.dlp[t]
                o.gemm_store(dp, dlp, 0, pk[f'wm2l{t}'], D, 1, n, D, dl, dmod[s0:s1], D, None, 0, None, None, 1.0, 0, 1)
                wgrad(dp, dlp, dl, st['omod'][s0:s1], D, D, f'model_to_latent_projs.{t}.weight', K = n)
            dneg = None
            if any_flow and self.clean:
                dneg = self.buf('dmod_neg', (S, D), F32)
                o.clean_flow_bwd(dmod, dneg, dv['row_token'], dv['cond_times'], dv['cond_row'], self.clean_eps, S, D)
            if any_flow:
                o.scatter_add_rows(d_out, dmod, dv['row_token'], S, D)
        g = self.buf('gx', (M, D), F32)
        o.rmsnorm_bwd(d_out, st['x_last'], self.P('transformer.norm.gamma'), g, self.G('transformer.norm.gamma'), M, D)

        hid = st['hid']
        dH = [self.buf(f'dH{l}', (M, D), F32) for l in range(self.depth + 1)]
        dskip = {}
        if nc > 0:
            dtab = self.buf('dtab', (nc, self.W * 3 * D), F32); dtab.zero_()
            dzg = self.buf('dzg', (nc, self.W * D), F32); dzg.zero_()
        dy = self.buf('dy', (M, D), BF16)
        du = self.buf('du', (M, D), F32)
        arws = self.buf('attn_res_ws', (int(o.lib.tfx_attn_residual_bwd_workspace_floats(M, D)),), F32)
        sc_stride = (self.depth + 2) * 3
        arsc = self.buf('attn_res_sc', (self.depth, M, self.depth + 2, 3), F32) if self.ares_deferred else None
        dxs = {}
        for i in reversed(range(self.depth)):
            L = st['layers'][i]
            pre = f'transformer.layers.{i}'
            lm = self.layer_maps[i]
            wA, wF = 2 * i, 2 * i + 1
            if self.ares_deferred:
                dxs[i] = g
                later = list(range(i + 1, self.depth))
                gam = [self.P(f'transformer.layers.{j}.3.norm_keys.gamma') for j in [i] + later]
                pqs = [self.P(f'transformer.layers.{j}.3.pseudo_queries') for j in [i] + later]
                o.attn_residual_bwd2(self._ptr_array(hid[:i + 2]), i + 2, 1, self._ptr_array(gam), self._ptr_array(pqs), self._ptr_array([dxs[j] for j in later] or [g]),
                                     self._ptr_array([arsc[j][0, i + 1] for j in later] or [g]), len(later), g, L['xr'], L['rlse'], dH[i + 1], arsc[i], sc_stride,
                                     self.G(f'{pre}.3.norm_keys.gamma'), self.G(f'{pre}.3.pseudo_queries'), arws, M, D)
            else:
              (o.attn_residual_bwd_h16 if self.hid_bf16 else o.attn_residual_bwd)(self._ptr_array(hid[:i + 2]), self._ptr_array(dH[:i + 2]), i + 2, self.P(f'{pre}.3.norm_keys.gamma'), self.P(f'{pre}.3.pseudo_queries'),
                                g, L['xr'], L['rlse'], self.G(f'{pre}.3.norm_keys.gamma'), self.G(f'{pre}.3.pseudo_queries'), arws, M, D, 1 if i == self.depth - 1 else 0)
            gx = dH[i + 1]
            o.resid_bwd(gx, L['yF'], cond_row, st['zg'][:, wF * D:] if nc > 0 else None, zg_ld, self.P(f'{pre}.2.layerscale'), dy,
                        dzg[:, wF * D:] if nc > 0 else None, zg_ld, self.G(f'{pre}.2.layerscale'), self.G(f'{pre}.2.fn.net.3.bias'), M, D)
            dh = self.buf('dh', (M, Ip), BF16)
            o.gemm_store(dy, D, 0, pk[f'w2{i}'], Ip, 1, M, Ip, D, None, 0, dh, Ip, None, None, 1.0, 0, 1)
            o.gemm_store(dy, D, 1, L['h'], Ip, 1, D, inner, M, self.gflat, 0, None, 0, None, lm['w2_rows'], 1.0, 1, ksplit(D, inner))
            dvg = self.buf('dvg', (M, 2 * Ip), BF16)
            rpb = self.ops.lib.tfx_geglu_bwd_rows_per_block()
            nblk = (M + rpb - 1) // rpb
            part = self.buf('geglu_part', (nblk, 2 * Ip), F32)
            if st['p_ff'] > 0.:
                o.geglu_bwd_drop(dh, L['vg'], dvg, M, Ip, None, None, part, st['drop_key'], st['p_ff'], i)
            else:
                o.geglu_bwd(dh, L['vg'], dvg, M, Ip, None, None, part)
            o.colsum_f32(part, 2 * Ip, nblk, 2 * Ip, lm['b1_cols'], self.gflat)
            o.gemm_store(dvg, 2 * Ip, 0, pk[f'w1{i}'], D, 1, M, D, 2 * Ip, du, D, None, 0, None, None, 1.0, 0, 1)
            o.gemm_store(dvg, 2 * Ip, 1, L['uF'], D, 1, 2 * Ip, D, M, self.gflat, 0, None, 0, None, lm['w1_rows'], 1.0, 1, ksplit(2 * Ip, D))
            o.adaln_bwd(du, L['x_b'], L['statsF'], cond_row, st['tab'][:, wF * 3 * D:] if nc > 0 else None, tab_ld, self.P(f'{pre}.2.layernorm_gamma'), gx,
                        dtab[:, wF * 3 * D:] if nc > 0 else None, tab_ld, self.G(f'{pre}.2.layernorm_gamma'), M, D)
            o.resid_bwd(gx, L['yA'], cond_row, st['zg'][:, wA * D:] if nc > 0 else None, zg_ld, self.P(f'{pre}.1.layerscale'), dy,
                        dzg[:, wA * D:] if nc > 0 else None, zg_ld, self.G(f'{pre}.1.layerscale'), None, M, D)
            dog = self.buf('dog', (M, HI), BF16)
            o.gemm_store(dy, D, 0, pk[f'wo{i}'], HI, 1, M, HI, D, None, 0, dog, HI, None, None, 1.0, 0, 1)
            wgrad(dy, D, D, L['att'], HI, HI, f'{pre}.1.fn.to_out.1.weight')
            dop = self.buf('dop', (M, HI), BF16); dsum_hm = self.buf('dsum_hm', (H, M), F32); dsum_mh = self.buf('dsum_mh', (M, H), F32)
            dq = self.buf('dq', (M, HI), F32); dk = self.buf('dk', (M, HI), F32)
            if self.laser:
                o.laser_bwd_prep(dog, L['o_l'], L['gates'], dop, dsum_hm, dsum_mh, dq, M, H)
            else:
                o.attn_bwd_prep(dog, L['att'], L['gates'], dop, dsum_hm, dsum_mh, dq, M, H)
            dqkvg = self.buf('dqkvg', (M, self.NQ), BF16)
            if i == self.depth - 1:
                dqkvg[:, 3 * HI + H:].zero_()
            fp = self.fastp[i]
            o.attn_bwd_tc(L['q'], L['k'], L['v_att'], dop, HI, HI, HI, HI, L['lse'], dsum_hm, dv['kv_limit'], dv['k2_kv0'], dv['k2_kvend'], dv['k2_q0'], dv['k2_qend'],
                          dv['k2_order'], int(rb.k2_kv0.shape[0]), dq, dk, dqkvg[:, 2 * HI:], self.NQ, M, H, self.scale, self.softcap, fp)
            o.attn_bwd(L['q'], L['k'], L['v_att'], dop, HI, HI, HI, HI, L['lse'], dsum_hm, dv['kv_limit'], dv['kt_kv0'], dv['kt_kvend'], dv['kt_q0'], dv['kt_qend'],
                       int(rb.kt_kv0.shape[0]), dq, dk, dqkvg[:, 2 * HI:], self.NQ, M, H, self.scale, self.softcap, fp)
            dv_cols = dqkvg[:, 2 * HI:]
            if self.laser:
                o.laser_v_bwd(dv_cols, self.NQ, L['v'], HI, M, H, self.laser_clamp)
            if self.vres:
                dv0 = self.buf('dv_first', (M, HI), F32)
                if i == self.depth - 1:
                    dv0.zero_()
                if i > 0:
                    o.vmix_bwd(dv_cols, self.NQ, L['v'], HI, st['layers'][0]['v'], HI, L['mixpre'], self.P(f'{pre}.1.fn.to_learned_value_residual.0.bias'), dv0,
                               dqkvg[:, 3 * HI + H:], self.NQ, M, H)
                    o.colsum_bf16(dqkvg[:, 3 * HI + H:], self.NQ, M, H, None, self.G(f'{pre}.1.fn.to_learned_value_residual.0.bias'))
                else:
                    dqkvg[:, 3 * HI + H:3 * HI + 2 * H].zero_()
                    o.add_f32_into_bf16(dv_cols, self.NQ, dv0, HI, M, HI)
            o.qk_bwd_pack(dq, dk, L['q'], L['k'], L['qk_inv'], self.P(f'{pre}.1.fn.q_norm.gamma'), self.P(f'{pre}.1.fn.k_norm.gamma'), dv['rope_pos'],
                          self.ws['rope_cs'], L['gates'], dsum_mh, dqkvg, self.NQ, self.G(f'{pre}.1.fn.q_norm.gamma'), self.G(f'{pre}.1.fn.k_norm.gamma'), M, H)
            o.gemm_store(dqkvg, self.NQ, 0, pk[f'qkvg{i}'], D, 1, M, D, self.NQ, du, D, None, 0, None, None, 1.0, 0, 1)
            o.gemm_store(dqkvg, self.NQ, 1, L['uA'], D, 1, self.NQ, D, M, self.gflat, 0, None, 0, None, lm['qkvg_rows'], 1.0, 1, ksplit(self.NQ, D))
            o.adaln_bwd(du, L['x_a'], L['statsA'], cond_row, st['tab'][:, wA * 3 * D:] if nc > 0 else None, tab_ld, self.P(f'{pre}.1.layernorm_gamma'), gx,
                        dtab[:, wA * 3 * D:] if nc > 0 else None, tab_ld, self.G(f'{pre}.1.layernorm_gamma'), M, D)
            if L['has_skip']:
                o.resid_bwd(gx, None, None, None, 0, None, dy, None, 0, None, None, M, D)
                wsk = pk[f'wskip{i}']
                gw = self.G(f'{pre}.0.weight')
                o.gemm_store(dy, D, 1, L['x_in_b'], D, 1, D, D, M, gw, 2 * D, None, 0, None, None, 1.0, 1, ksplit(D, D))
                o.gemm_store(dy, D, 1, L['skip_b'], D, 1, D, D, M, gw.view(-1)[D:], 2 * D, None, 0, None, None, 1.0, 1, ksplit(D, D))
                src = L['skip_src']
                assert src not in dskip
                dskip[src] = self.buf(f'dskip{src}', (M, D), F32)
                o.gemm_store(dy, D, 0, wsk[:, D:], 2 * D, 1, M, D, D, dskip[src], D, None, 0, None, None, 1.0, 0, 1)
                o.gemm_store(dy, D, 0, wsk, 2 * D, 1, M, D, D, gx, D, None, 0, None, None, 1.0, 1, 1)
            if i in dskip:
                o.axpy_f32(gx, dskip[i], 1.0, M * D)
            g = gx
            if bucket_cb is not None:
                bucket_cb(i)
        if self.ares_deferred:
            allj = list(range(self.depth))
            gam = [self.P(f'transformer.layers.{j}.3.norm_keys.gamma') for j in [0] + allj]
            pqs = [self.P(f'transformer.layers.{j}.3.pseudo_queries') for j in [0] + allj]
            o.attn_residual_bwd2(self._ptr_array(hid[:1]), 1, 0, self._ptr_array(gam), self._ptr_array(pqs), self._ptr_array([dxs[j] for j in allj]),
                                 self._ptr_array([arsc[j][0, 0] for j in allj]), len(allj), None, None, None, dH[0], None, sc_stride, None, None, None, M, D)
        o.axpy_f32(g, dH[0], 1.0, M * D)
        dmodtok = self.buf('dmodtok', (max(S, 1), D), BF16)
        o.embed_bwd(g, dv['text_id'], dv['slot'] if S > 0 else None, self.G('text_embed.weight'), dmodtok if S > 0 else None, M, D)
        if S > 0:
            if self.clean and dneg is not None:
                o.add_f32_into_bf16(dmodtok, D, dneg, D, S, D)
            for t, (tabs, coords) in st.get('posemb', {}).items():
                s0, s1 = rb.type_rows[t]
                nax = len(tabs)
                posemb_backward(dmodtok[s0:s1].float(), tabs, coords, self._posemb_params(t, nax), self._posemb_params(t, nax, grads = True))
            for t, (s0, s1) in enumerate(rb.type_rows):
                n = s1 - s0
                if n == 0 or f'latent_to_model_projs.{t}.weight' not in self.named:
                    continue
                dl, dlp = self.dls[t], self.dlp[t]
                o.gemm_store(dmodtok[s0:s1], D, 1, st['noised'][t], dlp, 1, D, dl, n, self.G(f'latent_to_model_projs.{t}.weight'), dl, None, 0, None, None, 1.0, 1,
                             max(1, min(ks, n // 128)))
                o.colsum_bf16(dmodtok[s0:s1], D, n, D, None, self.G(f'latent_to_model_projs.{t}.bias'))
        if nc > 0:
            W3 = self.W * 3 * D
            for w in range(self.W):
                o.table_op(dzg[:, w * D:], zg_ld, st['zg'][:, w * D:], zg_ld, dtab[:, w * 3 * D + 2 * D:], W3, None, 0, nc, D, 2)
            dtabb = self.buf('dtabb', (nc, W3), BF16)
            o.cast_bf16(dtab, dtabb, nc * W3)
            dcond = self.buf('dcond', (nc, 4 * D), F32)
            o.gemm_store(dtabb, W3, 0, pk['wfz'], 4 * D, 1, nc, 4 * D, W3, dcond, 4 * D, None, 0, None, None, 1.0, 0, 1)
            o.gemm_store(dtabb, W3, 1, st['cond'], 4 * D, 1, W3, 4 * D, nc, self.gflat, 0, None, 0, None, self.fz_rows, 1.0, 1, 1)
            bsum = self.buf('bsum', (W3,), F32); bsum.zero_()
            o.colsum_f32(dtab, W3, nc, W3, None, bsum)
            self.gflat.index_add_(0, self.fz_bias_idx, bsum)
            dcpre = self.buf('dcpre', (nc, 4 * D), BF16)
            o.table_op(dcond, 4 * D, st['cpre'], 4 * D, None, 0, dcpre, 4 * D, nc, 4 * D, 3)
            o.gemm_store(dcpre, 4 * D, 1, st['feats'], self.Kt, 1, 4 * D, D + 1, nc, self.gflat, 0, None, 0, None, self.wt_rows, 1.0, 1, 1)
            o.colsum_bf16(dcpre, 4 * D, nc, 4 * D, None, self.G('transformer.to_time_cond.1.bias'))

    def new_cache(self, n_slabs: int, cap: int) -> KVCache:
        self.ensure_attached()
        return KVCache(self, n_slabs, cap)

    def text_decoder(self, cache, S, **kw):
        from .decode import TextDecoder
        return TextDecoder(self, cache, S, **kw)

    def ode_solve(self, cache, rb, y, **kw):
        from .decode import ode_solve
        return ode_solve(self, cache, rb, y, **kw)

    def zero_grad(self):
        if not getattr(self, '_grads_clean', False):
            self.gflat.zero_()
        self._grads_clean = False

    def clip_grad_norm_(self, max_norm: float, pre_scale: float = 1.0):
        ss = self.buf('gnorm_ss', (1,), torch.float64)
        ss.zero_()
        n = self.gflat.numel()
        self.ops.grad_sumsq(self.gflat, n, ss)
        self.ops.clip_by_norm(self.gflat, n, ss, float(max_norm), float(pre_scale))
        return ss.sqrt() * pre_scale

    def ema_update(self, decay: float):
        if getattr(self, 'ema_flat', None) is None or self.ema_flat.numel() != self.flat.numel():
            self.ema_flat = self.flat.clone()
            return
        self.ops.ema_update(self.ema_flat, self.flat, self.flat.numel(), float(decay))

    def ema_state_dict(self):
        assert getattr(self, 'ema_flat', None) is not None, 'no EMA update has run yet'
        return {n: self.ema_flat[o:o + self.named[n].numel()].view(self.named[n].shape) for n, o in self.offs.items()}

    def adam_step(self, lr = 1e-3, betas = (0.9, 0.999), eps = 1e-8, weight_decay = 0., decoupled = False, grad_scale = 1.0, zero_grads = False, device_step = False):
        if self.exp_avg is None:
            self.exp_avg = torch.zeros_like(self.flat); self.exp_avg_sq = torch.zeros_like(self.flat)
        self.opt_step += 1
        step_dev = None
        if device_step:
            assert getattr(self, 'opt_step_dev', None) is not None, 'device_step needs engine.opt_step_dev (int32 [1] on the device)'
            step_dev = self.opt_step_dev
        self.ops.adam_step(self.flat, self.gflat, self.exp_avg, self.exp_avg_sq, self.flat.numel(), lr, betas[0], betas[1], eps, weight_decay, int(decoupled),
                           self.opt_step, grad_scale, int(zero_grads), step_dev)
        self._grads_clean = bool(zero_grads)
        self._dirty = True
```

Baseline: 933,600.

## Write GEMM store and GEGLU epilogues directly from registers via TMA tile stores

For the plain-store and GEGLU epilogues, accumulator fragments are now written straight from registers into swizzled output tiles in shared memory. Those tiles are then sent to global memory with TMA bulk tensor stores, replacing the f32 accumulator-tile round trip and per-warp staging copies. Dropping the accumulator tile frees shared memory, which buys a fifth pipeline stage for the store GEMM. The dropout keep mask is precomputed into shared memory, and the host ksplit tile count now matches the actual 128-wide tiles. The change adds tensor-map setup per launch and a fallback path for unaligned outputs, and it risks bulk-store waits serializing the epilogue.

```diff
diff --git a/transfusion_pytorch_b200/csrc/gemm_sm90.cuh b/transfusion_pytorch_b200/csrc/gemm_sm90.cuh
--- a/transfusion_pytorch_b200/csrc/gemm_sm90.cuh
+++ b/transfusion_pytorch_b200/csrc/gemm_sm90.cuh
@@ -40,20 +40,43 @@
   __nv_bfloat16* vg;
   __nv_bfloat16* h;
   DropParams drop;
+  int out_tma;
 };
+
+struct GemmOutMaps { CUtensorMap m[2]; };
 
 template <int EPI> struct GemmCfg {
   static constexpr int THREADS = 384;
-  static constexpr int STAGES = 4;
+  static constexpr int STAGES = EPI == 0 ? 5 : 4;
   static constexpr int A_BYTES = GEMM_BM * GEMM_BK * 2;
   static constexpr int B_BYTES = GEMM_BN * GEMM_BK * 2;
   static constexpr int STAGE_BYTES = A_BYTES + B_BYTES;
-  static constexpr int ACC_BYTES = GEMM_BM * GEMM_BN * 4;
-  static constexpr int STG_WARP = EPI == 2 ? 4096 + 2048 : 4096;
-  static constexpr int STAGING = (EPI >= 3 ? 8 : 4) * STG_WARP;
-  static constexpr int SMEM_BYTES = STAGES * STAGE_BYTES + ACC_BYTES + STAGING + 1024  + 256 ;
+  static constexpr bool ACC_TILE = EPI == 1 || EPI == 2;
+  static constexpr int ACC_BYTES = ACC_TILE ? GEMM_BM * GEMM_BN * 4 : 0;
+  static constexpr int STG_WARP = 4096 + 2048;
+  static constexpr int OUT_TILE = GEMM_BM * 128;
+  static constexpr int OUT_TILES = EPI >= 3 ? 3 : 2;
+  static constexpr int STAGING = ACC_TILE ? 4 * STG_WARP : 2 * OUT_TILES * OUT_TILE;
+  static constexpr int KEEP_BYTES = EPI == 4 ? 2 * 128 * 8 : 0;
+  static constexpr int SMEM_BYTES = STAGES * STAGE_BYTES + ACC_BYTES + STAGING + (EPI == 4 ? KEEP_BYTES : 1024 ) + 256 ;
   static_assert(SMEM_BYTES <= 227 * 1024, "shared memory of one block");
 };
+
+__device__ __forceinline__ uint32_t otile_bf16(int r, int c) { return r * 128 + ((((c >> 3) ^ (r & 7))) << 4) + (c & 7) * 2; }
+__device__ __forceinline__ uint32_t otile_f32(int r, int c) { return r * 128 + ((((c >> 2) ^ (r & 7))) << 4) + (c & 3) * 4; }
+
+template <class F>
+__device__ __forceinline__ void frag_for_each(const float (&d0)[64], const float (&d1)[64], int fr, int fc, F&& f) {
+#pragma unroll
+  for (int h = 0; h < 2; ++h)
+#pragma unroll
+    for (int q = 0; q < 16; ++q)
+#pragma unroll
+      for (int e = 0; e < 2; ++e) {
+        const float* d = h ? d1 : d0;
+        f(2 * h + e, h * 64 + fr + 8 * e, q, 8 * q + fc, d[4 * q + 2 * e], d[4 * q + 2 * e + 1]);
+      }
+}
 
 __device__ __forceinline__ uint32_t acc_off(int r, int col) { return r * 512 + ((((col >> 2) ^ (r & 7))) << 4) + (col & 3) * 4; }
 __device__ __forceinline__ void acc_ld32(const uint8_t* acc, int r, int col, uint32_t (&v)[32]) {
@@ -81,20 +104,10 @@
   return make_float2(gelu_erf(g.x) * v.x, gelu_erf(g.y) * v.y);
 }
 
-__device__ __forceinline__ void cp_async16_zfill(void* smem, const void* gmem, bool valid) {
-  const int sz = valid ? 16 : 0;
-  asm volatile("cp.async.cg.shared.global [%0], [%1], 16, %2;" ::"r"(smem_u32(smem)), "l"(gmem), "r"(sz) : "memory");
-}
-
 __device__ __forceinline__ uint32_t pack_bf16(float a, float b) {
   __nv_bfloat162 t = __floats2bfloat162_rn(a, b);
   return *reinterpret_cast<uint32_t*>(&t);
 }
-__device__ __forceinline__ float2 unpack2_bf16_(uint32_t w) {
-  __nv_bfloat162 t = *reinterpret_cast<__nv_bfloat162*>(&w);
-  return __bfloat1622float2(t);
-}
-
 template <int CH>
 __device__ __forceinline__ void stg_put(uint8_t* sw, int lane, const uint32_t* w) {
 #pragma unroll
@@ -134,12 +147,6 @@
   }
 }
 
-__device__ __forceinline__ void stg_put_pack(uint8_t* sw, int lane, const float* y) {
-#pragma unroll
-  for (int c = 0; c < 4; ++c)
-    *reinterpret_cast<uint4*>(sw + lane * 128 + ((c ^ (lane & 7)) << 4)) =
-        make_uint4(pack_bf16(y[8 * c], y[8 * c + 1]), pack_bf16(y[8 * c + 2], y[8 * c + 3]), pack_bf16(y[8 * c + 4], y[8 * c + 5]), pack_bf16(y[8 * c + 6], y[8 * c + 7]));
-}
 __device__ __forceinline__ void stg64_put(uint8_t* sw, int lane, const uint32_t* w) {
 #pragma unroll
   for (int c = 0; c < 4; ++c)
@@ -160,14 +167,6 @@
   }
 }
 
-__device__ __forceinline__ void stg64_store_rows(const uint8_t* sw, int lane, uint8_t* g, long long pitch, int rows_valid, const int* __restrict__ rows) {
-#pragma unroll
-  for (int it = 0; it < 4; ++it) {
-    const int row = it * 8 + (lane >> 2), ch = lane & 3;
-    if (row < rows_valid)
-      *reinterpret_cast<uint4*>(g + (long long)rows[row] * pitch + ch * 16) = *reinterpret_cast<const uint4*>(sw + row * 64 + ((ch ^ ((row >> 1) & 3)) << 4));
-  }
-}
 template <int CH>
 __device__ __forceinline__ void stg_store_rows(const uint8_t* sw, int lane, uint8_t* g, long long pitch, int rows_valid, const int* __restrict__ rows) {
   constexpr int RPI = 32 / CH;
@@ -179,9 +178,38 @@
   }
 }
 
+template <int ES, class Dst>
+__device__ __forceinline__ void otile_store_rows(const uint8_t* tile, int t128, int ncols, bool add, Dst&& dst) {
+  constexpr int EPC = 16 / ES;
+#pragma unroll 1
+  for (int it = 0; it < 8; ++it) {
+    const int r = it * 16 + (t128 >> 3), ch = t128 & 7;
+    uint8_t* g = dst(r);
+    if (g == nullptr || ch * EPC >= ncols) continue;
+    g += ch * 16;
+    const uint4 v = *reinterpret_cast<const uint4*>(tile + r * 128 + ((ch ^ (r & 7)) << 4));
+    if (ch * EPC + EPC <= ncols && (reinterpret_cast<uintptr_t>(g) & 15) == 0) {
+      if (add) asm volatile("red.global.add.v4.f32 [%0], {%1, %2, %3, %4};" ::"l"(g), "r"(v.x), "r"(v.y), "r"(v.z), "r"(v.w) : "memory");
+      else *reinterpret_cast<uint4*>(g) = v;
+    } else {
+      for (int e = 0; e < EPC && ch * EPC + e < ncols; ++e) {
+        const int wi = ES == 4 ? e : e >> 1;
+        const uint32_t w = wi == 0 ? v.x : wi == 1 ? v.y : wi == 2 ? v.z : v.w;
+        if (ES == 4) {
+          float* gf = reinterpret_cast<float*>(g) + e;
+          if (add) atomicAdd(gf, __uint_as_float(w)); else *gf = __uint_as_float(w);
+        } else {
+          reinterpret_cast<uint16_t*>(g)[e] = (uint16_t)(w >> (16 * (e & 1)));
+        }
+      }
+    }
+  }
+}
+
 template <bool A_MN, bool B_MN, int EPI, int CL>
 __global__ void __launch_bounds__(384, 1)
-gemm_sm90_kernel(const __grid_constant__ CUtensorMap tmA, const __grid_constant__ CUtensorMap tmA2, const __grid_constant__ CUtensorMap tmB, const GemmParams p) {
+gemm_sm90_kernel(const __grid_constant__ CUtensorMap tmA, const __grid_constant__ CUtensorMap tmA2, const __grid_constant__ CUtensorMap tmB,
+                 const __grid_constant__ GemmOutMaps om, const GemmParams p) {
   using Cfg = GemmCfg<EPI>;
   constexpr bool GEGLU = EPI == EPI_GEGLU || EPI == EPI_GEGLU_DROP;
   constexpr int BN = GEMM_BN;
@@ -192,7 +220,7 @@
   if (threadIdx.x == 0 && (smem_u32(smem) & 1023u) != 0) __trap();
   uint8_t* acc = smem + STAGES * Cfg::STAGE_BYTES;
   uint8_t* staging = acc + Cfg::ACC_BYTES;
-  uint64_t* bars = reinterpret_cast<uint64_t*>(staging + Cfg::STAGING);
+  uint64_t* bars = reinterpret_cast<uint64_t*>(staging + Cfg::STAGING + Cfg::KEEP_BYTES);
   uint64_t* full_bar = bars;
   uint64_t* empty_bar = bars + STAGES;
 
@@ -259,8 +287,14 @@
     constexpr int BAR_TILE = 1, BAR_MMA = 3, BAR_ACC = 5;
     const int cw = (warp >> 2) - 1;
     const int quad = warp & 3;
-    uint8_t* sw = staging + ((GEGLU ? 4 * cw : 0) + quad) * Cfg::STG_WARP;
-    const int erow = quad * 32 + lane;
+    const int fr = quad * 16 + (lane >> 2);
+    const int fc = 2 * (lane & 3);
+    const int t128 = threadIdx.x & 127;
+    const bool leader = t128 == 0;
+    uint8_t* const otile = staging + cw * Cfg::OUT_TILES * Cfg::OUT_TILE;
+    uint2* const keep_s = reinterpret_cast<uint2*>(staging + Cfg::STAGING) + 128 * cw;
+    auto otile_acquire = [&]() { if (leader) bulk_wait_read_all(); named_bar_sync(BAR_TILE + cw, 128); };
+    auto otile_release = [&]() { fence_proxy_async_smem(); named_bar_sync(BAR_TILE + cw, 128); };
     int stage = 0; uint32_t phase = 0;
     auto release = [&](int s) {
       __syncwarp();
@@ -284,6 +318,15 @@
         continue;
       }
       const bool has_next = item + item_stride < num_items;
+      if constexpr (EPI == EPI_GEGLU_DROP) {
+        const uint32_t k0 = __ldg(p.drop.key), k1 = __ldg(p.drop.key + 1);
+        const int own = lane & 3;
+        const uint32_t row = (uint32_t)(m_blk * GEMM_BM + (own >> 1) * 64 + fr + 8 * (own & 1));
+        uint32_t kw[2] = {0u, 0u};
+#pragma unroll
+        for (int q = 0; q < 8; ++q) kw[q >> 2] |= drop_keep8(p.drop, k0, k1, DROP_SITE_FFN, 0, row, (uint32_t)(n_blk * 8 + q)) << (8 * (q & 3));
+        keep_s[t128] = make_uint2(kw[0], kw[1]);
+      }
       if (nth > 0) named_bar_sync(BAR_MMA + cw, 256);
       float d0[64], d1[64];
 #pragma unroll
@@ -320,293 +363,284 @@
       wgmma_reg_fence(d1);
       if (prev_stage >= 0) release(prev_stage);
 
-      if (nth > 0) named_bar_sync(BAR_ACC + cw, 256);
-      {
-        const int r0 = quad * 16 + (lane >> 2);
+      const int row0 = m_blk * GEMM_BM;
+      const int col0 = n_blk * BN;
+
+      if constexpr (EPI == EPI_QKVG || EPI == EPI_RESID) {
+        if (nth > 0) named_bar_sync(BAR_ACC + cw, 256);
 #pragma unroll
         for (int q = 0; q < 16; ++q) {
-          const int c = 8 * q + 2 * (lane & 3);
-          *reinterpret_cast<float2*>(acc + acc_off(r0, c)) = make_float2(d0[4 * q], d0[4 * q + 1]);
-          *reinterpret_cast<float2*>(acc + acc_off(r0 + 8, c)) = make_float2(d0[4 * q + 2], d0[4 * q + 3]);
-          *reinterpret_cast<float2*>(acc + acc_off(r0 + 64, c)) = make_float2(d1[4 * q], d1[4 * q + 1]);
-          *reinterpret_cast<float2*>(acc + acc_off(r0 + 72, c)) = make_float2(d1[4 * q + 2], d1[4 * q + 3]);
-        }
-      }
-      named_bar_sync(BAR_TILE + cw, 128);
-
-      const int wrow0 = m_blk * GEMM_BM + quad * 32;
-      const int row = wrow0 + lane;
-      const bool row_ok = row < p.M;
-      const int rows_valid = min(32, p.M - wrow0);
-      const int col0 = n_blk * BN;
-      int qk_pos = 0;
-      if constexpr (EPI == EPI_QKVG) { qk_pos = row_ok ? p.rope_pos[row] : 0; }
-      if constexpr (EPI == EPI_RESID) { qk_pos = (row_ok && p.cond_row) ? p.cond_row[row] : -1; }
-
-      if constexpr (EPI == EPI_STORE) {
-        const bool f32_staged = p.out_f32 && (p.row_off || (p.ld_f32 & 3) == 0) && ((reinterpret_cast<uintptr_t>(p.out_f32) & 15) == 0);
-        const bool bf16_staged = p.out_bf16 && (p.ld_bf16 & 7) == 0 && ((reinterpret_cast<uintptr_t>(p.out_bf16) & 15) == 0);
-#pragma unroll 1
-        for (int c = 0; c < BN / 32; ++c) {
-          const int cbase = col0 + c * 32;
-          if (cbase >= p.N) break;
-          uint32_t r[32];
-          acc_ld32(acc, erow, c * 32, r);
-          const bool full = cbase + 32 <= p.N;
-          float v[32];
-#pragma unroll
-          for (int j = 0; j < 32; ++j) v[j] = __uint_as_float(r[j]);
-          if (p.alpha != 1.f) {
-#pragma unroll
-            for (int j = 0; j < 32; ++j) v[j] *= p.alpha;
-          }
-          if (p.bias) {
-            if (full) {
-#pragma unroll
-              for (int j = 0; j < 32; j += 4) { const float4 b = *reinterpret_cast<const float4*>(p.bias + cbase + j); v[j] += b.x; v[j + 1] += b.y; v[j + 2] += b.z; v[j + 3] += b.w; }
-            } else {
-              for (int j = 0; j < 32; ++j) if (cbase + j < p.N) v[j] += p.bias[cbase + j];
-            }
-          }
-          if (p.out_f32) {
-            if (full && f32_staged) {
-#pragma unroll
-              for (int j = 0; j < 32; ++j) r[j] = __float_as_uint(v[j]);
-              stg_put<8>(sw, lane, r);
-              __syncwarp();
-#pragma unroll
-              for (int it = 0; it < 8; ++it) {
-                const int rr = it * 4 + (lane >> 3), ch = lane & 7;
-                if (rr < rows_valid) {
-                  const long long off = p.row_off ? p.row_off[wrow0 + rr] : (long long)(wrow0 + rr) * p.ld_f32;
-                  if (off >= 0) {
-                    float* dst = p.out_f32 + off + cbase + ch * 4;
-                    const float4 t = *reinterpret_cast<const float4*>(sw + rr * 128 + ((ch ^ (rr & 7)) << 4));
-                    if ((reinterpret_cast<uintptr_t>(dst) & 15) == 0) {
-                      if (p.accumulate_f32) asm volatile("red.global.add.v4.f32 [%0], {%1, %2, %3, %4};" ::"l"(dst), "f"(t.x), "f"(t.y), "f"(t.z), "f"(t.w) : "memory");
-                      else *reinterpret_cast<float4*>(dst) = t;
-                    } else {
-                      if (p.accumulate_f32) { atomicAdd(dst, t.x); atomicAdd(dst + 1, t.y); atomicAdd(dst + 2, t.z); atomicAdd(dst + 3, t.w); }
-                      else { dst[0] = t.x; dst[1] = t.y; dst[2] = t.z; dst[3] = t.w; }
-                    }
-                  }
+          const int c = 8 * q + fc;
+          *reinterpret_cast<float2*>(acc + acc_off(fr, c)) = make_float2(d0[4 * q], d0[4 * q + 1]);
+          *reinterpret_cast<float2*>(acc + acc_off(fr + 8, c)) = make_float2(d0[4 * q + 2], d0[4 * q + 3]);
+          *reinterpret_cast<float2*>(acc + acc_off(fr + 64, c)) = make_float2(d1[4 * q], d1[4 * q + 1]);
+          *reinterpret_cast<float2*>(acc + acc_off(fr + 72, c)) = make_float2(d1[4 * q + 2], d1[4 * q + 3]);
+        }
+        named_bar_sync(BAR_TILE + cw, 128);
+        uint8_t* sw = staging + quad * Cfg::STG_WARP;
+        const int erow = quad * 32 + lane;
+        const int wrow0 = row0 + quad * 32;
+        const int row = wrow0 + lane;
+        const bool row_ok = row < p.M;
+        const int rows_valid = min(32, p.M - wrow0);
+        if constexpr (EPI == EPI_QKVG) {
+          const int qk_pos = row_ok ? p.rope_pos[row] : 0;
+          const int tps = p.H >> 1;
+          const int kind = n_blk / tps;
+          const int tis = n_blk - kind * tps;
+          const long long HI = (long long)p.H * 64;
+          if (kind <= 1) {
+            const float* gamma = kind == 0 ? p.q_gamma : p.k_gamma;
+            __nv_bfloat16* dstm = kind == 0 ? p.q : p.k;
+            const float2* cs = p.rope_cs + qk_pos;
+  #pragma unroll
+            for (int hh = 0; hh < 2; ++hh) {
+              uint32_t r0[32], r1[32];
+              acc_ld32(acc, erow, hh * 64, r0);
+              acc_ld32(acc, erow, hh * 64 + 32, r1);
+              float ss = 0.f;
+  #pragma unroll
+              for (int j = 0; j < 32; ++j) { float a = __uint_as_float(r0[j]), b = __uint_as_float(r1[j]); ss += a * a + b * b; }
+              const float inv = 1.f / fmaxf(sqrtf(ss), 1e-12f);
+              const int head = tis * 2 + hh;
+              if (row_ok) p.qk_inv[(long long)row * 2 * p.H + kind * p.H + head] = inv;
+              const float sc = inv * 8.f;
+              uint32_t outw[32];
+  #pragma unroll
+              for (int dh = 0; dh < 2; ++dh) {
+                uint32_t* rr = dh == 0 ? r0 : r1;
+  #pragma unroll
+                for (int i = 0; i < 16; ++i) {
+                  const int d0 = dh * 32 + 2 * i;
+                  const float2 gm = *reinterpret_cast<const float2*>(gamma + d0);
+                  const float y0 = __uint_as_float(rr[2 * i]) * sc * (gm.x + 1.f);
+                  const float y1 = __uint_as_float(rr[2 * i + 1]) * sc * (gm.y + 1.f);
+                  const float2 cc = cs[(long long)(dh * 16 + i) * p.rope_len];
+                  outw[dh * 16 + i] = pack_bf16(y0 * cc.x - y1 * cc.y, y1 * cc.x + y0 * cc.y);
                 }
               }
-              __syncwarp();
-            } else if (row_ok) {
-              const long long off = p.row_off ? p.row_off[row] : (long long)row * p.ld_f32;
-              if (off >= 0) {
-                float* dst = p.out_f32 + off + cbase;
-                for (int j = 0; j < 32; ++j)
-                  if (cbase + j < p.N) { if (p.accumulate_f32) atomicAdd(dst + j, v[j]); else dst[j] = v[j]; }
+              stg_put<8>(sw, lane, outw);
+              __syncwarp();
+              if (kind == 1 && p.kv_rows) stg_store_rows<8>(sw, lane, reinterpret_cast<uint8_t*>(dstm + head * 64), HI * 2, rows_valid, p.kv_rows + wrow0);
+              else stg_store<8>(sw, lane, reinterpret_cast<uint8_t*>(dstm + (long long)wrow0 * HI + head * 64), HI * 2, rows_valid);
+              __syncwarp();
+            }
+          } else if (kind == 2) {
+  #pragma unroll
+            for (int c = 0; c < 2; ++c) {
+              uint32_t r0[32], r1[32], w[32];
+              acc_ld32(acc, erow, c * 64, r0);
+              acc_ld32(acc, erow, c * 64 + 32, r1);
+  #pragma unroll
+              for (int j = 0; j < 16; ++j) {
+                w[j] = pack_bf16(__uint_as_float(r0[2 * j]), __uint_as_float(r0[2 * j + 1]));
+                w[16 + j] = pack_bf16(__uint_as_float(r1[2 * j]), __uint_as_float(r1[2 * j + 1]));
               }
-            }
-          }
-          if (p.out_bf16) {
-            if (full && bf16_staged) {
-              uint32_t w[16];
-#pragma unroll
-              for (int j = 0; j < 16; ++j) w[j] = pack_bf16(v[2 * j], v[2 * j + 1]);
-              stg_put<4>(sw, lane, w);
-              __syncwarp();
-              stg_store<4>(sw, lane, reinterpret_cast<uint8_t*>(p.out_bf16 + (long long)wrow0 * p.ld_bf16 + cbase), p.ld_bf16 * 2, rows_valid);
-              __syncwarp();
-            } else if (row_ok) {
-              __nv_bfloat16* dst = p.out_bf16 + (long long)row * p.ld_bf16 + cbase;
-              for (int j = 0; j < 32; ++j) if (cbase + j < p.N) dst[j] = __float2bfloat16(v[j]);
-            }
-          }
-        }
-      } else if constexpr (EPI == EPI_QKVG) {
-        const int tps = p.H >> 1;
-        const int kind = n_blk / tps;
-        const int tis = n_blk - kind * tps;
-        const long long HI = (long long)p.H * 64;
-        if (kind <= 1) {
-          const float* gamma = kind == 0 ? p.q_gamma : p.k_gamma;
-          __nv_bfloat16* dstm = kind == 0 ? p.q : p.k;
-          const float2* cs = p.rope_cs + qk_pos;
-#pragma unroll
-          for (int hh = 0; hh < 2; ++hh) {
-            uint32_t r0[32], r1[32];
-            acc_ld32(acc, erow, hh * 64, r0);
-            acc_ld32(acc, erow, hh * 64 + 32, r1);
-            float ss = 0.f;
-#pragma unroll
-            for (int j = 0; j < 32; ++j) { float a = __uint_as_float(r0[j]), b = __uint_as_float(r1[j]); ss += a * a + b * b; }
-            const float inv = 1.f / fmaxf(sqrtf(ss), 1e-12f);
-            const int head = tis * 2 + hh;
-            if (row_ok) p.qk_inv[(long long)row * 2 * p.H + kind * p.H + head] = inv;
-            const float sc = inv * 8.f;
-            uint32_t outw[32];
-#pragma unroll
-            for (int dh = 0; dh < 2; ++dh) {
-              uint32_t* rr = dh == 0 ? r0 : r1;
-#pragma unroll
-              for (int i = 0; i < 16; ++i) {
-                const int d0 = dh * 32 + 2 * i;
-                const float2 gm = *reinterpret_cast<const float2*>(gamma + d0);
-                const float y0 = __uint_as_float(rr[2 * i]) * sc * (gm.x + 1.f);
-                const float y1 = __uint_as_float(rr[2 * i + 1]) * sc * (gm.y + 1.f);
-                const float2 cc = cs[(long long)(dh * 16 + i) * p.rope_len];
-                outw[dh * 16 + i] = pack_bf16(y0 * cc.x - y1 * cc.y, y1 * cc.x + y0 * cc.y);
+              stg_put<8>(sw, lane, w);
+              __syncwarp();
+              if (p.kv_rows) stg_store_rows<8>(sw, lane, reinterpret_cast<uint8_t*>(p.v + tis * 128 + c * 64), HI * 2, rows_valid, p.kv_rows + wrow0);
+              else stg_store<8>(sw, lane, reinterpret_cast<uint8_t*>(p.v + (long long)wrow0 * HI + tis * 128 + c * 64), HI * 2, rows_valid);
+              __syncwarp();
+            }
+          } else {
+            uint32_t r[32];
+            acc_ld32(acc, erow, 0, r);
+            if (row_ok) {
+              float* dst = p.gates + (long long)row * p.H;
+  #pragma unroll
+              for (int j = 0; j < 32; ++j) if (j < p.H) dst[j] = __uint_as_float(r[j]);
+              if (p.mix_pre) {
+                float* dm = p.mix_pre + (long long)row * p.H;
+  #pragma unroll
+                for (int j = 0; j < 32; ++j) if (j >= p.H && j < 2 * p.H) dm[j - p.H] = __uint_as_float(r[j]);
               }
             }
-            stg_put<8>(sw, lane, outw);
+          }
+        } else {
+          const int crow = (row_ok && p.cond_row) ? p.cond_row[row] : -1;
+          const float* zrow = (p.zgate && crow >= 0) ? p.zgate + (long long)crow * p.zgate_ld : nullptr;
+          uint8_t* swb = sw + 4096;
+          uint4 xres[8];
+          auto fetch = [&](int sl) {
+            stg_fetch(lane, reinterpret_cast<const uint8_t*>(p.x_res + (long long)wrow0 * p.N + col0 + sl * 32), (long long)p.N * 4,
+                      col0 + sl * 32 < p.N ? rows_valid : 0, xres);
+          };
+          fetch(0);
+  #pragma unroll 1
+          for (int sl = 0; sl < BN / 32; ++sl) {
+            const int cbase = col0 + sl * 32;
+            if (cbase >= p.N) break;
             __syncwarp();
-            if (kind == 1 && p.kv_rows) stg_store_rows<8>(sw, lane, reinterpret_cast<uint8_t*>(dstm + head * 64), HI * 2, rows_valid, p.kv_rows + wrow0);
-            else stg_store<8>(sw, lane, reinterpret_cast<uint8_t*>(dstm + (long long)wrow0 * HI + head * 64), HI * 2, rows_valid);
+            stg_fill(sw, lane, xres);
+            if (sl + 1 < BN / 32) fetch(sl + 1);
+            uint32_t r[32];
+            acc_ld32(acc, erow, sl * 32, r);
+            float y[32];
+  #pragma unroll
+            for (int j = 0; j < 32; ++j) y[j] = __uint_as_float(r[j]);
+            if (p.bias) {
+  #pragma unroll
+              for (int j = 0; j < 32; j += 4) { const float4 b = *reinterpret_cast<const float4*>(p.bias + cbase + j); y[j] += b.x; y[j + 1] += b.y; y[j + 2] += b.z; y[j + 3] += b.w; }
+            }
+            if (p.y_bf16) {
+              stg64_put_pack(swb, lane, y);
+              __syncwarp();
+              stg64_store(swb, lane, reinterpret_cast<uint8_t*>(p.y_bf16 + (long long)wrow0 * p.N + cbase), (long long)p.N * 2, rows_valid);
+              __syncwarp();
+            }
+            {
+              uint32_t xrv[32];
+              __syncwarp();
+              stg_get<8>(sw, lane, xrv);
+              if (zrow) {
+  #pragma unroll
+                for (int j = 0; j < 32; j += 4) {
+                  const float4 s4 = *reinterpret_cast<const float4*>(zrow + cbase + j);
+                  y[j] = __uint_as_float(xrv[j]) + y[j] * s4.x; y[j + 1] = __uint_as_float(xrv[j + 1]) + y[j + 1] * s4.y;
+                  y[j + 2] = __uint_as_float(xrv[j + 2]) + y[j + 2] * s4.z; y[j + 3] = __uint_as_float(xrv[j + 3]) + y[j + 3] * s4.w;
+                }
+              } else if (p.ls) {
+  #pragma unroll
+                for (int j = 0; j < 32; j += 4) {
+                  const float4 s4 = *reinterpret_cast<const float4*>(p.ls + cbase + j);
+                  y[j] = __uint_as_float(xrv[j]) + y[j] * (s4.x + 1.f); y[j + 1] = __uint_as_float(xrv[j + 1]) + y[j + 1] * (s4.y + 1.f);
+                  y[j + 2] = __uint_as_float(xrv[j + 2]) + y[j + 2] * (s4.z + 1.f); y[j + 3] = __uint_as_float(xrv[j + 3]) + y[j + 3] * (s4.w + 1.f);
+                }
+              } else {
+  #pragma unroll
+                for (int j = 0; j < 32; ++j) y[j] += __uint_as_float(xrv[j]);
+              }
+            }
+            if (p.x_out)
+  #pragma unroll
+            for (int hfc = 0; hfc < 2; ++hfc) {
+              uint32_t w16[16];
+  #pragma unroll
+              for (int j = 0; j < 16; ++j) w16[j] = __float_as_uint(y[hfc * 16 + j]);
+              __syncwarp();
+              stg64_put(swb, lane, w16);
+              __syncwarp();
+              stg64_store(swb, lane, reinterpret_cast<uint8_t*>(p.x_out + (long long)wrow0 * p.N + cbase + hfc * 16), (long long)p.N * 4, rows_valid);
+            }
+            if (p.x_out_bf16) {
+              __syncwarp();
+              stg64_put_pack(swb, lane, y);
+              __syncwarp();
+              stg64_store(swb, lane, reinterpret_cast<uint8_t*>(p.x_out_bf16 + (long long)wrow0 * p.N + cbase), (long long)p.N * 2, rows_valid);
+            }
             __syncwarp();
           }
-        } else if (kind == 2) {
-#pragma unroll
-          for (int c = 0; c < 2; ++c) {
-            uint32_t r0[32], r1[32], w[32];
-            acc_ld32(acc, erow, c * 64, r0);
-            acc_ld32(acc, erow, c * 64 + 32, r1);
-#pragma unroll
-            for (int j = 0; j < 16; ++j) {
-              w[j] = pack_bf16(__uint_as_float(r0[2 * j]), __uint_as_float(r0[2 * j + 1]));
-              w[16 + j] = pack_bf16(__uint_as_float(r1[2 * j]), __uint_as_float(r1[2 * j + 1]));
-            }
-            stg_put<8>(sw, lane, w);
+        }
+        if (has_next) named_bar_arrive(BAR_ACC + (cw ^ 1), 256);
+      } else if constexpr (EPI == EPI_STORE) {
+        if (p.alpha != 1.f) {
+#pragma unroll
+          for (int i = 0; i < 64; ++i) { d0[i] *= p.alpha; d1[i] *= p.alpha; }
+        }
+        if (p.bias) {
+#pragma unroll
+          for (int q = 0; q < 16; ++q) {
+            const int c = col0 + 8 * q + fc;
+            const float b0 = c < p.N ? __ldg(p.bias + c) : 0.f, b1 = c + 1 < p.N ? __ldg(p.bias + c + 1) : 0.f;
+            d0[4 * q] += b0; d0[4 * q + 1] += b1; d0[4 * q + 2] += b0; d0[4 * q + 3] += b1;
+            d1[4 * q] += b0; d1[4 * q + 1] += b1; d1[4 * q + 2] += b0; d1[4 * q + 3] += b1;
+          }
+        }
+        if (p.out_f32) {
+#pragma unroll
+          for (int hc = 0; hc < 2; ++hc) {
+            if (col0 + hc * 64 >= p.N) break;
+            otile_acquire();
+            frag_for_each(d0, d1, fr, fc, [&](int, int r, int q, int c, float a, float b) {
+              if ((q >> 3) == hc)
+                *reinterpret_cast<float2*>(otile + ((q >> 2) & 1) * Cfg::OUT_TILE + otile_f32(r, c & 31)) = make_float2(a, b);
+            });
+            otile_release();
+#pragma unroll
+            for (int t = 0; t < 2; ++t) {
+              const int c = col0 + hc * 64 + t * 32;
+              if (c >= p.N) break;
+              if (p.out_tma & 1) {
+                if (leader) {
+                  if (p.accumulate_f32) tma_reduce_add_2d(&om.m[0], otile + t * Cfg::OUT_TILE, c, row0);
+                  else tma_store_2d(&om.m[0], otile + t * Cfg::OUT_TILE, c, row0);
+                }
+              } else {
+                otile_store_rows<4>(otile + t * Cfg::OUT_TILE, t128, p.N - c, p.accumulate_f32 != 0, [&](int r) -> uint8_t* {
+                  const int row = row0 + r;
+                  if (row >= p.M) return nullptr;
+                  const long long off = p.row_off ? p.row_off[row] : (long long)row * p.ld_f32;
+                  return off < 0 ? nullptr : reinterpret_cast<uint8_t*>(p.out_f32 + off + c);
+                });
+              }
+            }
+            if ((p.out_tma & 1) && leader) bulk_commit();
+          }
+        }
+        if (p.out_bf16) {
+          otile_acquire();
+          frag_for_each(d0, d1, fr, fc, [&](int, int r, int q, int c, float a, float b) {
+            *reinterpret_cast<uint32_t*>(otile + (q >> 3) * Cfg::OUT_TILE + otile_bf16(r, c & 63)) = pack_bf16(a, b);
+          });
+          otile_release();
+#pragma unroll
+          for (int t = 0; t < 2; ++t) {
+            const int c = col0 + t * 64;
+            if (c >= p.N) break;
+            if (p.out_tma & 2) {
+              if (leader) tma_store_2d(&om.m[1], otile + t * Cfg::OUT_TILE, c, row0);
+            } else {
+              otile_store_rows<2>(otile + t * Cfg::OUT_TILE, t128, p.N - c, false, [&](int r) -> uint8_t* {
+                const int row = row0 + r;
+                return row >= p.M ? nullptr : reinterpret_cast<uint8_t*>(p.out_bf16 + (long long)row * p.ld_bf16 + c);
+              });
+            }
+          }
+          if ((p.out_tma & 2) && leader) bulk_commit();
+        }
+      } else if constexpr (GEGLU) {
+        otile_acquire();
+#pragma unroll
+        for (int hq = 0; hq < 2; ++hq) {
+          uint32_t keep[4];
+          if constexpr (EPI == EPI_GEGLU_DROP) {
             __syncwarp();
-            if (p.kv_rows) stg_store_rows<8>(sw, lane, reinterpret_cast<uint8_t*>(p.v + tis * 128 + c * 64), HI * 2, rows_valid, p.kv_rows + wrow0);
-            else stg_store<8>(sw, lane, reinterpret_cast<uint8_t*>(p.v + (long long)wrow0 * HI + tis * 128 + c * 64), HI * 2, rows_valid);
-            __syncwarp();
-          }
-        } else {
-          uint32_t r[32];
-          acc_ld32(acc, erow, 0, r);
-          if (row_ok) {
-            float* dst = p.gates + (long long)row * p.H;
-#pragma unroll
-            for (int j = 0; j < 32; ++j) if (j < p.H) dst[j] = __uint_as_float(r[j]);
-            if (p.mix_pre) {
-              float* dm = p.mix_pre + (long long)row * p.H;
-#pragma unroll
-              for (int j = 0; j < 32; ++j) if (j >= p.H && j < 2 * p.H) dm[j - p.H] = __uint_as_float(r[j]);
-            }
-          }
-        }
-      } else if constexpr (EPI == EPI_RESID) {
-        const int crow = qk_pos;
-        const float* zrow = (p.zgate && crow >= 0) ? p.zgate + (long long)crow * p.zgate_ld : nullptr;
-        uint8_t* swb = sw + 4096;
-        uint4 xres[8];
-        auto fetch = [&](int sl) {
-          stg_fetch(lane, reinterpret_cast<const uint8_t*>(p.x_res + (long long)wrow0 * p.N + col0 + sl * 32), (long long)p.N * 4,
-                    col0 + sl * 32 < p.N ? rows_valid : 0, xres);
-        };
-        fetch(0);
-#pragma unroll 1
-        for (int sl = 0; sl < BN / 32; ++sl) {
-          const int cbase = col0 + sl * 32;
-          if (cbase >= p.N) break;
-          __syncwarp();
-          stg_fill(sw, lane, xres);
-          if (sl + 1 < BN / 32) fetch(sl + 1);
-          uint32_t r[32];
-          acc_ld32(acc, erow, sl * 32, r);
-          float y[32];
-#pragma unroll
-          for (int j = 0; j < 32; ++j) y[j] = __uint_as_float(r[j]);
-          if (p.bias) {
-#pragma unroll
-            for (int j = 0; j < 32; j += 4) { const float4 b = *reinterpret_cast<const float4*>(p.bias + cbase + j); y[j] += b.x; y[j + 1] += b.y; y[j + 2] += b.z; y[j + 3] += b.w; }
-          }
-          if (p.y_bf16) {
-            stg64_put_pack(swb, lane, y);
-            __syncwarp();
-            stg64_store(swb, lane, reinterpret_cast<uint8_t*>(p.y_bf16 + (long long)wrow0 * p.N + cbase), (long long)p.N * 2, rows_valid);
-            __syncwarp();
-          }
-          {
-            uint32_t xrv[32];
-            __syncwarp();
-            stg_get<8>(sw, lane, xrv);
-            if (zrow) {
-#pragma unroll
-              for (int j = 0; j < 32; j += 4) {
-                const float4 s4 = *reinterpret_cast<const float4*>(zrow + cbase + j);
-                y[j] = __uint_as_float(xrv[j]) + y[j] * s4.x; y[j + 1] = __uint_as_float(xrv[j + 1]) + y[j + 1] * s4.y;
-                y[j + 2] = __uint_as_float(xrv[j + 2]) + y[j + 2] * s4.z; y[j + 3] = __uint_as_float(xrv[j + 3]) + y[j + 3] * s4.w;
+#pragma unroll
+            for (int i = 0; i < 4; ++i) { const uint2 k = keep_s[(t128 & ~3) | i]; keep[i] = hq ? k.y : k.x; }
+          }
+#pragma unroll
+          for (int q = 4 * hq; q < 4 * hq + 4; ++q) {
+            const int c = 8 * q + fc;
+            const float2 bv = make_float2(__ldg(p.bias + col0 + c), __ldg(p.bias + col0 + c + 1));
+            const float2 bg = make_float2(__ldg(p.bias + col0 + 64 + c), __ldg(p.bias + col0 + 64 + c + 1));
+#pragma unroll
+            for (int i = 0; i < 4; ++i) {
+              float* d = i < 2 ? d0 : d1;
+              const int e = 2 * (i & 1), r = (i >> 1) * 64 + fr + 8 * (i & 1);
+              const float2 v = make_float2(d[4 * q + e] + bv.x, d[4 * q + e + 1] + bv.y);
+              const float2 g = make_float2(d[4 * (q + 8) + e] + bg.x, d[4 * (q + 8) + e + 1] + bg.y);
+              *reinterpret_cast<uint32_t*>(otile + otile_bf16(r, c)) = pack_bf16(v.x, v.y);
+              *reinterpret_cast<uint32_t*>(otile + Cfg::OUT_TILE + otile_bf16(r, c)) = pack_bf16(g.x, g.y);
+              float2 o = geglu_pair(g, v);
+              if constexpr (EPI == EPI_GEGLU_DROP) {
+                const uint32_t kb = keep[i] >> (8 * (q & 3) + fc);
+                o.x = kb & 1u ? o.x * p.drop.scale : 0.f;
+                o.y = kb & 2u ? o.y * p.drop.scale : 0.f;
               }
-            } else if (p.ls) {
-#pragma unroll
-              for (int j = 0; j < 32; j += 4) {
-                const float4 s4 = *reinterpret_cast<const float4*>(p.ls + cbase + j);
-                y[j] = __uint_as_float(xrv[j]) + y[j] * (s4.x + 1.f); y[j + 1] = __uint_as_float(xrv[j + 1]) + y[j + 1] * (s4.y + 1.f);
-                y[j + 2] = __uint_as_float(xrv[j + 2]) + y[j + 2] * (s4.z + 1.f); y[j + 3] = __uint_as_float(xrv[j + 3]) + y[j + 3] * (s4.w + 1.f);
-              }
-            } else {
-#pragma unroll
-              for (int j = 0; j < 32; ++j) y[j] += __uint_as_float(xrv[j]);
-            }
-          }
-          if (p.x_out)
-#pragma unroll
-          for (int hfc = 0; hfc < 2; ++hfc) {
-            uint32_t w16[16];
-#pragma unroll
-            for (int j = 0; j < 16; ++j) w16[j] = __float_as_uint(y[hfc * 16 + j]);
-            __syncwarp();
-            stg64_put(swb, lane, w16);
-            __syncwarp();
-            stg64_store(swb, lane, reinterpret_cast<uint8_t*>(p.x_out + (long long)wrow0 * p.N + cbase + hfc * 16), (long long)p.N * 4, rows_valid);
-          }
-          if (p.x_out_bf16) {
-            __syncwarp();
-            stg64_put_pack(swb, lane, y);
-            __syncwarp();
-            stg64_store(swb, lane, reinterpret_cast<uint8_t*>(p.x_out_bf16 + (long long)wrow0 * p.N + cbase), (long long)p.N * 2, rows_valid);
-          }
-          __syncwarp();
-        }
-      } else if constexpr (GEGLU) {
-        uint32_t keep[2] = {0u, 0u};
-        if constexpr (EPI == EPI_GEGLU_DROP) {
-          const uint32_t k0 = __ldg(p.drop.key), k1 = __ldg(p.drop.key + 1);
-#pragma unroll
-          for (int q = 0; q < 8; ++q) keep[q >> 2] |= drop_keep8(p.drop, k0, k1, DROP_SITE_FFN, 0, (uint32_t)row, (uint32_t)(n_blk * 8 + q)) << (8 * (q & 3));
-        }
-        uint32_t ra[4][32];
-#pragma unroll
-        for (int q = 0; q < 4; ++q) acc_ld32(acc, erow, q * 32, ra[q]);
-        if (has_next) named_bar_arrive(BAR_ACC + (cw ^ 1), 256);
-#pragma unroll
-        for (int c = 0; c < 2; ++c) {
-          const int cv = col0 + c * 32, cg = cv + 64;
-          if (cv >= p.N) break;
-          float v[32], g[32];
-#pragma unroll
-          for (int j = 0; j < 32; ++j) { v[j] = __uint_as_float(ra[c][j]) + p.bias[cv + j]; g[j] = __uint_as_float(ra[2 + c][j]) + p.bias[cg + j]; }
-          __syncwarp();
-          stg64_put_pack(sw, lane, v);
-          __syncwarp();
-          stg64_store(sw, lane, reinterpret_cast<uint8_t*>(p.vg + (long long)wrow0 * p.N + cv), (long long)p.N * 2, rows_valid);
-          __syncwarp();
-          stg64_put_pack(sw, lane, g);
-          __syncwarp();
-          stg64_store(sw, lane, reinterpret_cast<uint8_t*>(p.vg + (long long)wrow0 * p.N + cg), (long long)p.N * 2, rows_valid);
-#pragma unroll
-          for (int j = 0; j < 32; j += 2) {
-            const float2 o = geglu_pair(make_float2(g[j], g[j + 1]), make_float2(v[j], v[j + 1]));
-            g[j] = o.x; g[j + 1] = o.y;
-          }
-          if constexpr (EPI == EPI_GEGLU_DROP) {
-#pragma unroll
-            for (int j = 0; j < 32; ++j) g[j] = (keep[c] >> j) & 1u ? g[j] * p.drop.scale : 0.f;
-          }
-          __syncwarp();
-          stg64_put_pack(sw, lane, g);
-          __syncwarp();
-          stg64_store(sw, lane, reinterpret_cast<uint8_t*>(p.h + (long long)wrow0 * (p.N / 2) + n_blk * 64 + c * 32), (long long)p.N, rows_valid);
-          __syncwarp();
+              *reinterpret_cast<uint32_t*>(otile + 2 * Cfg::OUT_TILE + otile_bf16(r, c)) = pack_bf16(o.x, o.y);
+            }
+          }
+        }
+        otile_release();
+        if (leader) {
+          tma_store_2d(&om.m[0], otile, col0, row0);
+          tma_store_2d(&om.m[0], otile + Cfg::OUT_TILE, col0 + 64, row0);
+          tma_store_2d(&om.m[1], otile + 2 * Cfg::OUT_TILE, n_blk * 64, row0);
+          bulk_commit();
         }
       }
-      if (!GEGLU && has_next) named_bar_arrive(BAR_ACC + (cw ^ 1), 256);
     }
+    if constexpr (!Cfg::ACC_TILE) { if (leader) bulk_wait_all(); }
   }
   if constexpr (CL > 1) {
     __syncthreads();
@@ -640,6 +674,21 @@
                    CU_TENSOR_MAP_INTERLEAVE_NONE, CU_TENSOR_MAP_SWIZZLE_128B, CU_TENSOR_MAP_L2_PROMOTION_L2_256B,
                    CU_TENSOR_MAP_FLOAT_OOB_FILL_NONE);
   return r == CUDA_SUCCESS ? 0 : -(int)r - 1000;
+}
+
+inline int make_tmap_out(CUtensorMap* tm, const void* ptr, int esize, long long inner, long long outer, long long ld) {
+  PFN_encodeTiled enc = get_encode_fn();
+  if (!enc) return -1;
+  cuuint64_t dims[2] = {(cuuint64_t)inner, (cuuint64_t)outer};
+  cuuint64_t strides[1] = {(cuuint64_t)ld * esize};
+  cuuint32_t box[2] = {(cuuint32_t)(128 / esize), (cuuint32_t)GEMM_BM};
+  cuuint32_t estr[2] = {1, 1};
+  CUresult r = enc(tm, esize == 4 ? CU_TENSOR_MAP_DATA_TYPE_FLOAT32 : CU_TENSOR_MAP_DATA_TYPE_BFLOAT16, 2, const_cast<void*>(ptr), dims, strides, box, estr,
+                   CU_TENSOR_MAP_INTERLEAVE_NONE, CU_TENSOR_MAP_SWIZZLE_128B, CU_TENSOR_MAP_L2_PROMOTION_NONE, CU_TENSOR_MAP_FLOAT_OOB_FILL_NONE);
+  return r == CUDA_SUCCESS ? 0 : -(int)r - 1000;
+}
+inline bool tma_storable(const void* ptr, long long ld, long long inner, int esize) {
+  return (reinterpret_cast<uintptr_t>(ptr) & 15) == 0 && (ld * esize) % 16 == 0 && (inner * esize) % 16 == 0;
 }
 
 struct GemmOperand {
@@ -677,6 +726,16 @@
   const int m_tiles = (p.M + GEMM_BM - 1) / GEMM_BM, n_tiles = (p.N + GEMM_BN - 1) / GEMM_BN;
   const int items = m_tiles * n_tiles * p.k_splits;
   if (items <= 0) return 0;
+  GemmOutMaps om;
+  memset(&om, 0, sizeof(om));
+  p.out_tma = 0;
+  if constexpr (EPI == EPI_STORE) {
+    if (p.out_f32 && !p.row_off && tma_storable(p.out_f32, p.ld_f32, p.N, 4) && make_tmap_out(&om.m[0], p.out_f32, 4, p.N, p.M, p.ld_f32) == 0) p.out_tma |= 1;
+    if (p.out_bf16 && tma_storable(p.out_bf16, p.ld_bf16, p.N, 2) && make_tmap_out(&om.m[1], p.out_bf16, 2, p.N, p.M, p.ld_bf16) == 0) p.out_tma |= 2;
+  } else if constexpr (EPI == EPI_GEGLU || EPI == EPI_GEGLU_DROP) {
+    rc = make_tmap_out(&om.m[0], p.vg, 2, p.N, p.M, p.N); if (rc) return rc;
+    rc = make_tmap_out(&om.m[1], p.h, 2, p.N / 2, p.M, p.N / 2); if (rc) return rc;
+  }
   const int mode = gemm_cluster_mode_ref();
   const int kb_item = ((p.K + GEMM_BK - 1) / GEMM_BK + p.k_splits - 1) / p.k_splits;
   const bool paired = mode == 2 || (mode == 3 && m_tiles >= 2 && kb_item >= 16 && items >= 2 * num_sms);
@@ -701,7 +760,7 @@
     const int pair_items = ((m_tiles + 1) / 2) * n_tiles * p.k_splits;
     const int clusters = pair_items < max_clusters ? pair_items : max_clusters;
     cfg.gridDim = dim3(2 * clusters);
-    return cudaLaunchKernelEx(&cfg, kern, tmA, tmA2, tmB, p) == cudaSuccess ? 0 : -3;
+    return cudaLaunchKernelEx(&cfg, kern, tmA, tmA2, tmB, om, p) == cudaSuccess ? 0 : -3;
   }
   auto kern = gemm_sm90_kernel<A_MN, B_MN, EPI, 1>;
   static bool attr_set = false;
@@ -710,7 +769,7 @@
     attr_set = true;
   }
   const int grid = items < num_sms ? items : num_sms;
-  kern<<<grid, Cfg::THREADS, Cfg::SMEM_BYTES, stream>>>(tmA, tmA2, tmB, p);
+  kern<<<grid, Cfg::THREADS, Cfg::SMEM_BYTES, stream>>>(tmA, tmA2, tmB, om, p);
   return cudaGetLastError() == cudaSuccess ? 0 : -3;
 }
 
diff --git a/transfusion_pytorch_b200/csrc/sm90_ptx.cuh b/transfusion_pytorch_b200/csrc/sm90_ptx.cuh
--- a/transfusion_pytorch_b200/csrc/sm90_ptx.cuh
+++ b/transfusion_pytorch_b200/csrc/sm90_ptx.cuh
@@ -65,6 +65,10 @@
 }
 __device__ __forceinline__ void tma_reduce_add_2d(const CUtensorMap* m, const void* smem, int c0, int c1) {
   asm volatile("cp.reduce.async.bulk.tensor.2d.global.shared::cta.add.tile.bulk_group [%0, {%2, %3}], [%1];"
+               ::"l"(reinterpret_cast<uint64_t>(m)), "r"(smem_u32(smem)), "r"(c0), "r"(c1) : "memory");
+}
+__device__ __forceinline__ void tma_store_2d(const CUtensorMap* m, const void* smem, int c0, int c1) {
+  asm volatile("cp.async.bulk.tensor.2d.global.shared::cta.bulk_group [%0, {%2, %3}], [%1];"
                ::"l"(reinterpret_cast<uint64_t>(m)), "r"(smem_u32(smem)), "r"(c0), "r"(c1) : "memory");
 }
 __device__ __forceinline__ void bulk_commit() { asm volatile("cp.async.bulk.commit_group;" ::: "memory"); }
diff --git a/transfusion_pytorch_b200/engine.py b/transfusion_pytorch_b200/engine.py
--- a/transfusion_pytorch_b200/engine.py
+++ b/transfusion_pytorch_b200/engine.py
@@ -631,7 +631,7 @@
         ks = max(1, min(64, M // 2048))
         sms = torch.cuda.get_device_properties(self.device).multi_processor_count
         def ksplit(n_out, n_in, K = M):
-            tiles = ((n_out + 127) // 128) * ((n_in + 255) // 256 if (n_in % 256 == 0 or n_in >= 1024) else (n_in + 127) // 128)
+            tiles = ((n_out + 127) // 128) * ((n_in + 127) // 128)
             best, best_eff = 1, 0.0
             for s in range(1, 65):
                 if K // s < 1024 and s > 1:
```

New measurement: 951,600, median of 6. +1.9%, better.
